# karfly/learnable-triangulation-pytorch

Hardware: AMD Instinct MI355X
Metric: multi-view samples/sec (4-view vol-softmax forward) (higher is better)
Workload: dtype bf16; 1 GPU; BASELINE config 2: volumetric-softmax forward, 4 views 384x384, 64^3 voxel cube, ResNet-152, random-init weights; per_gpu_batch=64, global_batch=64, parallelism=batch-sharded replicas x1, no data-path collective, hip_graph=True, self_launched=False

## Files before the change

include/lt_hip.h:

```cpp
#ifndef LT_HIP_H
#define LT_HIP_H

#include <stddef.h>
#include <stdint.h>

#ifdef __cplusplus
extern "C" {
#endif

#define LT_ABI_VERSION 1

enum { LT_F32 = 0, LT_BF16 = 1,
       LT_FP8 = 2  };
enum { LT_OK = 0, LT_ERR_INVALID = -1, LT_ERR_UNSUPPORTED = -2, LT_ERR_LAUNCH = -3 };

enum { LT_AGG_SUM = 0, LT_AGG_MAX = 1, LT_AGG_SOFTMAX = 2, LT_AGG_CONF = 3,
       LT_AGG_CONF_NORM = 4  };

enum {
    LT_EPI_RELU_PRE = 1,
    LT_EPI_RELU_POST = 2,
    LT_EPI_STORE_F32 = 4,
    LT_EPI_SIGMOID = 8,
    LT_EPI_RES_F32 = 64,
    LT_BN_FROZEN = 32,
    LT_BN_Y_BF16 = 128,
    LT_ACT_BF16 = 256
};

const char* lt_last_error(void);
int lt_abi_version(void);
int lt_device_info(int* cu_count, int* lds_per_cu, char* arch, int arch_len);

#define LT_CONV_MAX_PHASES 8

typedef struct lt_conv_phase {
    const void* weight;
    const int32_t* taps;
    int32_t ntaps;
    int32_t out_off[3];
    const void* weight_frag;
    int32_t weight_frag_layout;
} lt_conv_phase;

typedef struct lt_conv_desc {
    int32_t dtype;
    int32_t N, D, H, W, Cin;
    int32_t Do, Ho, Wo;
    int32_t stride[3], pad[3];
    int32_t OD, OH, OW;
    int32_t out_stride[3];
    int32_t Cout, ldc;
    int32_t cout_pad, k_pad;
    int32_t nphase;
    int32_t flags;
    int32_t tile;
    int32_t stages;
    lt_conv_phase phase[LT_CONV_MAX_PHASES];
} lt_conv_desc;

int lt_conv_pack_weights(const void* weight, int32_t cout_pad, int32_t k_pad, void* packed, void* stream);
int lt_conv_pack_weights_t32(const void* weight, int32_t cout_pad, int32_t k_pad, int32_t cin, int32_t ntaps, void* packed,
                             void* stream);
int lt_conv_pack_weights32(const void* weight, int32_t cout_pad, int32_t k_pad, void* packed, void* stream);

enum { LT_TILE_AUTO = 0,
       LT_TILE_128x128 = 1, LT_TILE_128x64 = 2, LT_TILE_256x32 = 3, LT_TILE_256x16 = 4, LT_TILE_64x64 = 5,
       LT_TILE2_128x128 = 11, LT_TILE2_128x64 = 12, LT_TILE2_256x32 = 13, LT_TILE2_256x16 = 14, LT_TILE2_64x64 = 15,
       LT_TILE_HALO = 20,
       LT_TILE3_288 = 30,
       LT_TILE_DIRECT = 99  };

int lt_conv_fwd(const lt_conv_desc* desc, const void* x, const float* bias, const float* scale, const float* shift,
                const void* residual, void* y, void* stream);
typedef struct lt_conv_skip {
    const void* x;
    int32_t cin;
    const void* weight_frag;
} lt_conv_skip;
int lt_conv_skip_fwd(const lt_conv_desc* desc, const void* x, const float* bias, const float* scale, const float* shift,
                     const lt_conv_skip* skip, void* y, void* stream);
typedef struct lt_conv_cat2 {
    const void* x;
    int32_t cin, H, W, stride;
} lt_conv_cat2;
int lt_conv_cat2_fwd(const lt_conv_desc* desc, const void* x, const lt_conv_cat2* second, const float* bias, const float* scale, const float* shift,
                     const void* residual, void* y, void* stream);
int lt_conv_cout_pad(int32_t cout);
int32_t lt_conv_chunk_samples(int32_t N, int64_t per_sample);

typedef struct lt_wshape {
    int32_t nd;
    int64_t s[5];
} lt_wshape;
int lt_sel_conv_skip(int32_t dtype, const int32_t x[5], const lt_wshape* w, const int32_t skip_x[5], const lt_wshape* skip_w);
int lt_sel_halo7_col(int32_t dtype, const int32_t x[5]);
int lt_sel_conv_cat2(int32_t dtype, const int32_t t2[5], const lt_wshape* w_expand, const int32_t x[5], const lt_wshape* w_down, int32_t stride_down);
int lt_sel_splitk_slices(const lt_conv_desc* d, const lt_wshape* w, int32_t transposed);
int lt_sel_bottleneck(int32_t dtype, const int32_t x[5], const lt_wshape w[3], const int32_t strides[3]);
int lt_sel_bottleneck_ds(int32_t dtype, const int32_t x[5], const lt_wshape w[3], const int32_t strides[3], const lt_wshape* w_down, int32_t stride_down);
int lt_sel_expand_reduce(int32_t dtype, const int32_t t2[5], const int32_t res[5], const lt_wshape* w_expand, const lt_wshape* w_reduce);
int lt_sel_stem_pool(int32_t dtype, const int32_t x[5], const lt_wshape* w, int32_t stride, int32_t pad, const int32_t pool[3]);
int lt_sel_pwchain(int32_t dtype, const int32_t x[5], int32_t nlayers, const lt_wshape* w);
int lt_sel_frag_layout(const lt_conv_desc* d, const lt_wshape* w, int32_t transposed, int32_t has_residual);

int lt_maxpool_fwd(int32_t dtype, const void* x, void* y, int32_t N, int32_t D, int32_t H, int32_t W, int32_t C,
                   const int32_t k[3], const int32_t s[3], const int32_t p[3], void* stream);

int lt_global_avgpool(int32_t dtype, const void* x, void* y, int32_t N, int32_t HW, int32_t C, void* stream);

int lt_nchw_to_nhwc(int32_t dtype, const float* x, void* y, int32_t N, int32_t C, int32_t HW, int32_t c_pad, void* stream);
int lt_nhwc_to_nchw_f32(int32_t dtype, const void* x, float* y, int32_t N, int32_t C, int32_t HW, int32_t ld, void* stream);

int lt_splitk_reduce(int32_t dtype, const float* partial, int32_t S, int64_t N, int64_t rows_per_sample, int32_t C, const float* bias,
                     const float* scale, const float* shift, const void* residual, void* y, int32_t flags, void* stream);

int lt_coord_volumes(const float* pos, const float* center, const float* rot, float step, int32_t B, int32_t V,
                     int32_t cmu_transfer, float* coords, void* stream);
int lt_rotate_points(const float* x, const float* rot, float* y, int64_t n, void* stream);

int lt_unproject_fwd(int32_t dtype, const void* feats, const float* proj, const float* coords, const float* conf,
                     void* out, int32_t B, int32_t NV, int32_t C, int32_t h, int32_t w, int32_t v0, int32_t v1,
                     int32_t v2, int32_t agg, void* stream);
int lt_unproject_grid_fwd(int32_t dtype, const void* feats, const float* proj, const float* pos, const float* center, const float* rot,
                          float step, int32_t cmu_transfer, float* coords_out, const float* conf, void* out, int32_t B, int32_t NV,
                          int32_t C, int32_t h, int32_t w, int32_t V, int32_t agg, void* stream);
int lt_unproject_masked_fwd(int32_t dtype, const void* feats, const float* proj, const float* coords, const float* conf, const uint8_t* view_mask,
                            void* out, int32_t B, int32_t NV, int32_t C, int32_t h, int32_t w, int32_t v0, int32_t v1, int32_t v2, int32_t agg,
                            void* stream);
int lt_unproject_grid_masked_fwd(int32_t dtype, const void* feats, const float* proj, const float* pos, const float* center, const float* rot,
                                 float step, int32_t cmu_transfer, float* coords_out, const float* conf, const uint8_t* view_mask, void* out,
                                 int32_t B, int32_t NV, int32_t C, int32_t h, int32_t w, int32_t V, int32_t agg, void* stream);
enum { LT_KIND_MPII = 0, LT_KIND_COCO = 1 };
int lt_cuboid_from_keypoints(const float* keypoints_3d, int32_t B, int32_t J, int32_t kind, double cuboid_side, float* pos, float* center,
                             void* stream);

size_t lt_softargmax3d_workspace(int32_t B, int32_t J, int64_t nvox);
int lt_softargmax3d_fwd(const float* logits, const float* coords, float mult, int32_t softmax, int32_t channels_last,
                        int32_t ld, float* kp, float* probs, int32_t B, int32_t J, int64_t nvox, void* workspace,
                        void* stream);
size_t lt_softargmax3d_stats_workspace(int32_t B, int32_t J, int64_t nvox);
int lt_softargmax3d_stats_fwd(const float* logits, const float* coords, float mult, int32_t softmax, int32_t channels_last, int32_t ld,
                              float* kp, float* probs, float* stats, int32_t* peak_index, int32_t B, int32_t J, int64_t nvox, void* workspace,
                              void* stream);

int lt_softargmax2d_fwd(const float* heatmaps, float mult, int32_t softmax, float* coords, float* probs, int32_t NJ,
                        int32_t h, int32_t w, void* stream);
int lt_softargmax2d_stats_fwd(const float* heatmaps, float mult, int32_t softmax, float* coords, float* probs, float* stats, int32_t* peak_index,
                              int32_t NJ, int32_t h, int32_t w, void* stream);
int lt_softargmax2d_bwd(const float* probs, const float* coords, const float* grad_coords, float mult, int32_t softmax, float* grad_heatmaps,
                        int32_t NJ, int32_t h, int32_t w, void* stream);
int lt_triangulate_dlt_bwd(const float* proj, const float* points, const float* conf, const float* grad_out, float* grad_points, float* grad_conf,
                           int32_t B, int32_t NV, int32_t J, void* stream);

size_t lt_unproject_bwd_workspace(int32_t B, int32_t NV, int32_t C, int32_t v0, int32_t v1, int32_t v2);
int lt_unproject_bwd(int32_t dtype, const void* feats, const float* proj, const float* coords, const float* conf, const float* grad_out,
                     float* grad_feats, float* grad_conf, int32_t B, int32_t NV, int32_t C, int32_t h, int32_t w, int32_t v0, int32_t v1,
                     int32_t v2, int32_t agg, void* workspace, size_t workspace_bytes, void* stream);
int lt_unproject_masked_bwd(int32_t dtype, const void* feats, const float* proj, const float* coords, const float* conf, const uint8_t* view_mask,
                            const float* grad_out, float* grad_feats, float* grad_conf, int32_t B, int32_t NV, int32_t C, int32_t h, int32_t w,
                            int32_t v0, int32_t v1, int32_t v2, int32_t agg, void* workspace, size_t workspace_bytes, void* stream);
int lt_softargmax3d_bwd(const float* probs, const float* coords, const float* kp, const float* grad_kp, const int32_t* gp_idx,
                        const float* gp_val, float multiplier, int32_t softmax, int32_t channels_last, float* grad_logits, int32_t B,
                        int32_t J, int64_t nvox, void* stream);
int lt_softargmax3d_bwd_dense(const float* probs, const float* coords, const float* kp, const float* grad_kp, const int32_t* gp_idx,
                              const float* gp_val, const float* gp_dense, float* workspace_bj, float multiplier, int32_t softmax,
                              int32_t channels_last, float* grad_logits, int32_t B, int32_t J, int64_t nvox, void* stream);
int lt_volumetric_ce_fwd(const float* coords, const float* probs, const float* keypoints_gt, const float* validity, float* terms,
                         int32_t* idx, float* grad_val, int32_t B, int32_t J, int64_t nvox, void* stream);
size_t lt_bn_stats_workspace(int64_t rows, int32_t C);
int lt_bn_stats_fwd(int32_t dtype, const void* x, int64_t rows, int32_t C, float* mean, float* var, float* running_mean,
                    float* running_var, float momentum, void* workspace, void* stream);

int lt_bn_act_fwd(const void* y , const float* mean, const float* var, const float* gamma, const float* beta, const void* residual, void* z,
                  void* z_bf16 , int64_t rows, int32_t C, float eps,
                  int32_t flags, void* stream);
size_t lt_bn_act_bwd_workspace(int64_t rows, int32_t C);
int lt_bn_act_bwd(const void* dz, const void* y , const void* residual, const float* mean, const float* var, const float* gamma, const float* beta,
                  void* dy, void* dy_bf16 , float* dgamma, float* dbeta, void* dres, int32_t accumulate_res,
                  int64_t rows, int32_t C, float eps, int32_t flags, void* workspace, void* stream);
int lt_act_bwd(const void* dz, const void* z, const void* residual, void* dy, void* dres, int32_t accumulate_res, int64_t total, int32_t flags,
               void* stream);
size_t lt_channel_sum_workspace(int64_t rows, int32_t C);
// ... 40 lines not shown
                       void* stream);
int lt_adam_step(float* param, const float* grad, float* exp_avg, float* exp_avg_sq, int64_t n, float lr, double beta1, double beta2, float eps,
                 float weight_decay, int32_t step, void* stream);

int lt_triangulate_dlt(const float* proj, const float* points, const float* conf, float* out, int32_t B, int32_t NV,
                       int32_t J, void* stream);
int lt_alg_tail_fwd(const float* keypoints_hm, const float* conf_raw, int32_t ld_conf, const float* proj, float scale_x, float scale_y,
                    float* keypoints_2d, float* confidences, float* keypoints_3d, int32_t B, int32_t NV, int32_t J, void* stream);
int lt_alg_tail_masked_fwd(const float* keypoints_hm, const float* conf_raw, int32_t ld_conf, const float* proj, float scale_x, float scale_y,
                           const uint8_t* view_mask, float* keypoints_2d, float* confidences, float* keypoints_3d, int32_t B, int32_t NV,
                           int32_t J, void* stream);
int lt_alg_tail_stats_fwd(const float* keypoints_hm, const float* conf_raw, int32_t ld_conf, const float* proj, float scale_x, float scale_y,
                          const uint8_t* view_mask, const float* stats2d, float* keypoints_2d, float* confidences, float* keypoints_3d,
                          float* cov2d_img, float* reproj_err, float* cov3d, int32_t B, int32_t NV, int32_t J, void* stream);
int lt_triangulate_dlt_stats(const float* proj, const float* points, const float* conf, const float* cov2d, const uint8_t* view_mask, float* out,
                             float* reproj_err, float* cov3d, int32_t B, int32_t NV, int32_t J, void* stream);

int lt_heatmap_argmax_nchw_f32(const float* heatmaps, int32_t ld, float* heatmaps_nchw, int64_t* indices, int64_t* keypoints,
                               int32_t N, int32_t J, int32_t h, int32_t w, int32_t image_h, int32_t image_w, void* stream);
int lt_triangulate_ransac(const float* proj, const int64_t* points, const int32_t* pairs, int32_t n_iters, double eps, int32_t direct_opt,
                          float* out_kp3d, uint8_t* out_inliers, int32_t B, int32_t NV, int32_t J, void* stream);

int lt_crop_resize_u8(const uint8_t* src, int64_t src_bytes, const int64_t* desc, const int64_t* desc_host, int32_t N, int32_t H, int32_t W,
                      const float* lut, float* out, void* stream);

int lt_undistort_crop_resize_u8(const uint8_t* src, int64_t src_bytes, const int64_t* desc, const int64_t* desc_host, const int16_t* maps,
                                int64_t maps_bytes, int32_t N, int32_t H, int32_t W, const float* lut, float* out, void* stream);

#define LT_PWCHAIN_MAX 3
typedef struct {
    int32_t dtype;
    int32_t nlayers;
    int64_t rows;
    int32_t cin;
    int32_t ldy;
    int32_t cout[LT_PWCHAIN_MAX];
    int32_t k_pad[LT_PWCHAIN_MAX];
    int32_t flags[LT_PWCHAIN_MAX];
    const void* weight[LT_PWCHAIN_MAX];
    const float* bias[LT_PWCHAIN_MAX];
    const float* scale[LT_PWCHAIN_MAX];
    const float* shift[LT_PWCHAIN_MAX];
    int64_t plane;
} lt_pwchain_desc;
int lt_pwchain_fwd(const lt_pwchain_desc* desc, const void* x, void* y, void* stream);

typedef struct {
    int32_t dtype;
    int32_t N, H, W;
    int32_t Cin, Cout;
    const void* weight;
    const float* bias;
    const float* scale;
    const float* shift;
    int32_t x_layout;
} lt_stem_desc;
size_t lt_stem_packed_bytes(void);
int lt_stem_pack_weights(const void* weight, int32_t k_pad, void* packed, void* stream);
int lt_stem_pool_fwd(const lt_stem_desc* desc, const void* x, void* y, void* stream);

typedef struct {
    int32_t dtype;
    int32_t N, H, W;
    int32_t C, P;
    const void* weight[3];
    const float* bias[3];
    const float* scale[3];
    const float* shift[3];
} lt_bneck_desc;
int lt_bottleneck_fwd(const lt_bneck_desc* desc, const void* x, void* y, void* stream);

typedef struct {
    int32_t dtype;
    int32_t N, H, W;
    int32_t Cin, P, C;
    const void* weight[4];
    const float* scale[4];
    const float* shift[4];
} lt_bneck_ds_desc;
int lt_bottleneck_ds_fwd(const lt_bneck_ds_desc* desc, const void* x, void* y, void* stream);

typedef struct {
    int32_t dtype;
    int32_t C, P;
    int64_t M;
    const void* weight[2];
    const float* scale[2];
    const float* shift[2];
    const float* consts;
} lt_xr_desc;
int lt_expand_reduce_fwd(const lt_xr_desc* desc, const void* t2, const void* residual, void* y, void* t1_next, void* stream);

int lt_graph_begin(void* stream);
int lt_graph_end(void* stream, void** graph_exec_out);
int lt_graph_launch(void* graph_exec, void* stream);
int lt_graph_destroy(void* graph_exec);
int lt_event_create(void** ev_out);
int lt_event_record(void* ev, void* stream);
int lt_event_elapsed_ms(void* ev_start, void* ev_stop, float* ms_out);
int lt_event_destroy(void* ev);

typedef struct lt_plan lt_plan;
typedef struct lt_named_tensor {
    const char* name;
    const float* data;
    int32_t ndim;
    int64_t shape[5];
} lt_named_tensor;
typedef struct lt_vol_plan_config {
    int32_t dtype;
    int32_t num_layers;
    int32_t style_caffe;
    int32_t num_joints;
    int32_t B, NV, H, W;
    int32_t volume_size;
    double cuboid_side;
    double volume_multiplier;
    int32_t volume_softmax;
    int32_t aggregation;
    int32_t transfer_cmu_to_human36m;
    int32_t use_graph;
} lt_vol_plan_config;
typedef struct lt_plan_info_t {
    int32_t launches;
    int32_t heatmap_h, heatmap_w;
    double flops;
    int64_t bytes_allocated;
    int32_t n_expand_reduce, n_bottleneck, n_bottleneck_ds, n_conv_cat2, n_conv2d_halo, n_pwchain, n_stem_pool, n_splitk, n_conv_skip;
    int32_t graph_captured;
    const float* logits;
    int32_t logits_planar;
} lt_plan_info_t;
int lt_plan_create_vol(const lt_vol_plan_config* cfg, const lt_named_tensor* weights, int32_t nweights, lt_plan** plan_out);
int lt_plan_forward_vol(lt_plan* plan, const float* images, const double* K_host, const double* R_host, const double* t_host, const double* base_points_host,
                        const double* rot_host, float* keypoints_3d, float* volumes, float* features, float* coord_volumes, float* vol_confidences, void* stream);
enum { LT_MODEL_ALG = 1, LT_MODEL_RANSAC = 2 };
typedef struct lt_alg_plan_config {
    int32_t model;
    int32_t dtype;
    int32_t num_layers;
    int32_t style_caffe;
    int32_t num_joints;
    int32_t B, NV, H, W;
    int32_t use_confidences;
    int32_t heatmap_softmax;
    double heatmap_multiplier;
    int32_t direct_optimization;
    double reprojection_error_epsilon;
    int32_t use_graph;
} lt_alg_plan_config;
int lt_plan_create_alg(const lt_alg_plan_config* cfg, const lt_named_tensor* weights, int32_t nweights, lt_plan** plan_out);
int lt_plan_forward_alg(lt_plan* plan, const float* images, const float* proj, float* keypoints_3d, void* keypoints_2d, float* heatmaps,
                        float* confidences, void* stream);
typedef struct lt_cascade_plan_config {
    lt_alg_plan_config alg;
    lt_vol_plan_config vol;
    int32_t kind;
} lt_cascade_plan_config;
int lt_plan_create_cascade(const lt_cascade_plan_config* cfg, const lt_named_tensor* alg_weights, int32_t n_alg, const lt_named_tensor* vol_weights,
                           int32_t n_vol, lt_plan** plan_out);
int lt_plan_forward_cascade(lt_plan* plan, const float* images, const double* K_host, const double* R_host, const double* t_host, const double* rot_host,
                            float* keypoints_3d, float* alg_keypoints_3d, float* base_points, float* volumes, float* features, float* coord_volumes,
                            float* vol_confidences, void* stream);
int lt_plan_set_view_mask(lt_plan* plan, const uint8_t* mask_host);
int lt_plan_set_keypoint_stats(lt_plan* plan, float* stats_dev, int32_t* peak_index_dev);
int lt_plan_set_alg_keypoint_stats(lt_plan* plan, float* stats2d_dev, int32_t* peak_index_dev, float* cov2d_img_dev, float* reproj_err_dev,
                                   float* cov3d_dev);
int lt_plan_info(const lt_plan* plan, lt_plan_info_t* info);
void lt_plan_destroy(lt_plan* plan);

#ifdef __cplusplus
}
#endif
#endif
```

learnable-triangulation-pytorch_amd/csrc/bneck.hip:

```cpp
#include <stdlib.h>

#include <type_traits>

#include "wave_prims.h"

using namespace lt;

namespace {

__device__ uint4 g_zero_page_b[2];

#ifdef LT_BNECK_TRACE
#define LT_BNECK_TRACE_WG 4096
__device__ unsigned long long g_bneck_trace[LT_BNECK_TRACE_WG * 4 * 8];
#define BN_STAMP(k)                                                                                                  \
    do {                                                                                                             \
        if (blockIdx.x < LT_BNECK_TRACE_WG && lane == 0) g_bneck_trace[(blockIdx.x * 4 + wave) * 8 + (k)] = clock64(); \
    } while (0)
#else
#define BN_STAMP(k)
#endif

struct BneckArgs {
    const bf16_t* x;
// ... 623 lines not shown
                }
                const int slot = (4 * cb + 2 * q + hk) ^ fsw(n31);
                *(uint4*)((lptr_t)(size_t)(lds0 + T2_OFF + px * RB + slot * 16)) = make_uint4(o[0], o[1], o[2], o[3]);
            }
        }
    }
    __syncthreads();

    {
        const unsigned a2 = lds0 + T2_OFF + n31 * RB + ((hk ^ fsw(n31)) << 4);
        unsigned xd[NPB][2];
#pragma unroll
        for (int pb = 0; pb < NPB; ++pb) {
            const int hpc = (2 * pb + prr + 1) * HPI + pcc + 1;
#pragma unroll
            for (int s2 = 0; s2 < 2; ++s2) xd[pb][s2] = lds0 + XS_OFF + hpc * 64 + (((2 * s2 + hk) ^ swz64(hpc)) << 4);
        }
        f32x16 acc[NPB], accd[NPB];
        static_for<0, NU3>([&](auto uc) {
            constexpr int u = decltype(uc)::value;
            constexpr int q = u / NUQ, k = u % NUQ;
            const int ob = wave + 4 * q;
            if constexpr (k == 0) {
#pragma unroll
                for (int pb = 0; pb < NPB; ++pb)
#pragma unroll
                    for (int e = 0; e < 16; ++e) { acc[pb][e] = 0.f; accd[pb][e] = 0.f; }
            }
            if constexpr (u + WD3 < NU3) wf3[(u + WD3) % (WD3 + 1)] = load_w3(u + WD3);
            V16 xb[NPB];
            if constexpr (k < GD) {
#pragma unroll
                for (int pb = 0; pb < NPB; ++pb) xb[pb].u = *(const uint4*)((lptr_t)(size_t)(xd[pb][k & 1] + (k >> 1) * STAGE));
#pragma unroll
                for (int pb = 0; pb < NPB; ++pb)
                    accd[pb] = __builtin_amdgcn_mfma_f32_32x32x16_bf16(wf3[u % (WD3 + 1)].h, xb[pb].h, accd[pb], 0, 0, 0);
            } else {
                constexpr int g = k - GD;
#pragma unroll
                for (int pb = 0; pb < NPB; ++pb) xb[pb].u = *(const uint4*)((lptr_t)(size_t)((a2 ^ (g << 5)) + pb * 32 * RB));
#pragma unroll
                for (int pb = 0; pb < NPB; ++pb)
                    acc[pb] = __builtin_amdgcn_mfma_f32_32x32x16_bf16(wf3[u % (WD3 + 1)].h, xb[pb].h, acc[pb], 0, 0, 0);
            }
            __builtin_amdgcn_sched_barrier(0);
            if constexpr (k == NUQ - 1) {
#pragma unroll
                for (int j = 0; j < 2; ++j) {
                    float esc[8], esf[8], dsc[8], dsf[8];
#pragma unroll
                    for (int e = 0; e < 8; ++e) {
                        esc[e] = csel(cst3, 128 * q, 8 * j + e);
                        esf[e] = csel(cst3, 128 * q + 32, 8 * j + e);
                        dsc[e] = csel(cst3, 128 * q + 64, 8 * j + e);
                        dsf[e] = csel(cst3, 128 * q + 96, 8 * j + e);
                    }
#pragma unroll
                    for (int pb = 0; pb < NPB; ++pb) {
                        unsigned o[4];
#pragma unroll
                        for (int d = 0; d < 4; ++d) {
                            const int e = 2 * d;
                            const float r0 = accd[pb][8 * j + e] * dsc[e] + dsf[e], r1 = accd[pb][8 * j + e + 1] * dsc[e + 1] + dsf[e + 1];
                            const float v0 = fmaxf(acc[pb][8 * j + e] * esc[e] + esf[e] + r0, 0.f);
                            const float v1 = fmaxf(acc[pb][8 * j + e + 1] * esc[e + 1] + esf[e + 1] + r1, 0.f);
                            o[d] = pack_bf16x2(v0, v1);
                        }
                        *(uint4*)(a.y + poff[pb] + 32 * ob + 16 * j) = make_uint4(o[0], o[1], o[2], o[3]);
                    }
                }
            }
        });
    }
}

int launch_bneck_ds(const BneckDsArgs& a, hipStream_t s) {
    constexpr int lds = 180 * 128 + 2 * 180 * 64 + 128 * 128;
    static_assert(lds <= 80 * 1024, "two workgroups per CU");
    auto kern = bneck_ds_kernel<64, 64, 256>;
    LT_OPT_IN_LDS(kern, lds);
    const long long nblk = (long long)a.N * a.tiles_x * a.tiles_y;
    hipLaunchKernelGGL(kern, dim3((unsigned)nblk), dim3(256), lds, s, a);
    LT_CHECK_LAUNCH("lt_bottleneck_ds_fwd");
    return LT_OK;
}

}

#ifdef LT_BNECK_TRACE
extern "C" int lt_bneck_trace_read(void* host, int nbytes) {
    return (int)hipMemcpyFromSymbol(host, HIP_SYMBOL(g_bneck_trace), nbytes, 0, hipMemcpyDeviceToHost);
}
#endif

extern "C" int lt_bottleneck_fwd(const lt_bneck_desc* d, const void* x, void* y, void* stream) {
    LT_REQUIRE(d && x && y, LT_ERR_INVALID, "lt_bottleneck_fwd: null argument");
    LT_REQUIRE(x != y, LT_ERR_INVALID, "lt_bottleneck_fwd: in-place is not possible (neighbouring tiles read each other's halo)");
    LT_REQUIRE(d->dtype == LT_BF16, LT_ERR_UNSUPPORTED, "lt_bottleneck_fwd: bf16 only");
    LT_REQUIRE((d->C == 256 && d->P == 64) || (d->C == 512 && d->P == 128), LT_ERR_UNSUPPORTED,
               "lt_bottleneck_fwd: widths %d / %d (256 / 64 and 512 / 128: the identity blocks of ResNet layer1 / layer2)", d->C, d->P);
    LT_REQUIRE(d->N > 0 && d->H > 0 && d->W > 0 && d->H % 8 == 0 && d->W % 16 == 0, LT_ERR_UNSUPPORTED,
               "lt_bottleneck_fwd: map %d x %d (8 x 16 pixel tiles)", d->H, d->W);
    LT_REQUIRE((long long)d->N * d->H * d->W * d->C < (1ll << 31), LT_ERR_UNSUPPORTED, "lt_bottleneck_fwd: 32-bit element offsets");
    BneckArgs a;
    a.x = (const bf16_t*)x;
    a.y = (bf16_t*)y;
    a.w1 = (const bf16_t*)d->weight[0];
    a.w2 = (const bf16_t*)d->weight[1];
    a.w3 = (const bf16_t*)d->weight[2];
    for (int i = 0; i < 3; ++i) {
        LT_REQUIRE(d->weight[i] && d->scale[i] && d->shift[i], LT_ERR_INVALID, "lt_bottleneck_fwd: layer %d: null weight / scale / shift", i);
        a.bias[i] = d->bias[i];
        a.scale[i] = d->scale[i];
        a.shift[i] = d->shift[i];
    }
    a.N = d->N; a.H = d->H; a.W = d->W;
    a.tiles_x = d->W / 16; a.tiles_y = d->H / 8;
    hipStream_t s = (hipStream_t)stream;
#ifndef LT_BNECK_HELD64
#define LT_BNECK_HELD64 2
#endif
#ifndef LT_BNECK_HELD128
#define LT_BNECK_HELD128 1
#endif
    if (d->P == 64) return launch_bneck<256, 64, 4, LT_BNECK_HELD64>(a, s);
    return launch_bneck<512, 128, 3, LT_BNECK_HELD128>(a, s);
}

extern "C" int lt_bottleneck_ds_fwd(const lt_bneck_ds_desc* d, const void* x, void* y, void* stream) {
    LT_REQUIRE(d && x && y, LT_ERR_INVALID, "lt_bottleneck_ds_fwd: null argument");
    LT_REQUIRE(x != y, LT_ERR_INVALID, "lt_bottleneck_ds_fwd: in-place is not possible");
    LT_REQUIRE(d->dtype == LT_BF16, LT_ERR_UNSUPPORTED, "lt_bottleneck_ds_fwd: bf16 only");
    LT_REQUIRE(d->Cin == 64 && d->P == 64 && d->C == 256, LT_ERR_UNSUPPORTED,
               "lt_bottleneck_ds_fwd: widths %d -> %d -> %d (64 -> 64 -> 256: the first block of ResNet layer1)", d->Cin, d->P, d->C);
    LT_REQUIRE(d->N > 0 && d->H > 0 && d->W > 0 && d->H % 8 == 0 && d->W % 16 == 0, LT_ERR_UNSUPPORTED,
               "lt_bottleneck_ds_fwd: map %d x %d (8 x 16 pixel tiles)", d->H, d->W);
    LT_REQUIRE((long long)d->N * d->H * d->W * d->C < (1ll << 31), LT_ERR_UNSUPPORTED, "lt_bottleneck_ds_fwd: 32-bit element offsets");
    BneckDsArgs a;
    a.x = (const bf16_t*)x;
    a.y = (bf16_t*)y;
    for (int i = 0; i < 4; ++i) {
        LT_REQUIRE(d->weight[i] && d->scale[i] && d->shift[i], LT_ERR_INVALID, "lt_bottleneck_ds_fwd: layer %d: null weight / scale / shift", i);
        a.scale[i] = d->scale[i];
        a.shift[i] = d->shift[i];
    }
    a.w1 = (const bf16_t*)d->weight[0];
    a.w2 = (const bf16_t*)d->weight[1];
    a.w3 = (const bf16_t*)d->weight[2];
    a.wd = (const bf16_t*)d->weight[3];
    a.N = d->N; a.H = d->H; a.W = d->W;
    a.tiles_x = d->W / 16; a.tiles_y = d->H / 8;
    return launch_bneck_ds(a, (hipStream_t)stream);
}
```

learnable-triangulation-pytorch_amd/csrc/plan.hip:

```cpp
#include <math.h>
#include <stdlib.h>
#include <string.h>

#include <array>
#include <deque>
#include <functional>
#include <map>
#include <string>
#include <unordered_map>
#include <vector>

#include "lt_common.h"

using namespace lt;

namespace {

#define PL_TRY(call)                   \
    do {                               \
        const int rc_ = (call);        \
        if (rc_ != LT_OK) return rc_;  \
    } while (0)
#define PL_HIP(call)                                                        \
    do {                                                                    \
// ... 142 lines not shown
        const int o = (dims[i] - 1) * 2 - 2 * pd[i] + ks[i] + output_padding;
        LT_REQUIRE(o == 2 * dims[i], LT_ERR_UNSUPPORTED, "plan: a transposed convolution must exactly double the size (k = 4, p = 1 / k = 2, p = 0)");
        outs[i] = o;
    }
    const int cp = cout_pad_of(cout);
    struct DimPhase { int phi; std::vector<std::pair<int, int>> taps; };
    auto dim_phases = [&](int i) {
        std::vector<DimPhase> res;
        if (!nd3 && i == 0) { res.push_back({0, {{0, 0}}}); return res; }
        for (int phi = 0; phi < 2; ++phi) {
            DimPhase dp; dp.phi = phi;
            for (int kk = 0; kk < ks[i]; ++kk)
                if (floormod(phi + pd[i] - kk, 2) == 0) dp.taps.push_back({kk, floordiv(phi + pd[i] - kk, 2)});
            res.push_back(dp);
        }
        return res;
    };
    const int64_t ktot = (int64_t)kd * kh * kw;
    struct Raw { std::vector<std::pair<std::vector<float>, int>> dummy; };
    std::vector<PhaseSpec> phases;
    std::vector<std::vector<int>> phase_k;
    int ntaps_max = 0;
    for (const DimPhase& A : dim_phases(0))
        for (const DimPhase& Bp : dim_phases(1))
            for (const DimPhase& Cp : dim_phases(2)) {
                PhaseSpec ph; std::vector<int> kidx;
                for (auto& ta : A.taps)
                    for (auto& tb : Bp.taps)
                        for (auto& tc : Cp.taps) {
                            const int da = ta.second, db = tb.second, dc = tc.second;
                            ph.taps.push_back(da); ph.taps.push_back(db); ph.taps.push_back(dc); ph.taps.push_back(((da * Hh + db) * W + dc) * cin);
                            kidx.push_back((ta.first * kh + tb.first) * kw + tc.first);
                        }
                if (kidx.empty()) { ph.taps = {0, 0, 0, 0}; kidx.push_back(-1); }
                ph.ntaps = (int)kidx.size();
                ph.off[0] = A.phi; ph.off[1] = Bp.phi; ph.off[2] = Cp.phi;
                if (ph.ntaps > ntaps_max) ntaps_max = ph.ntaps;
                phases.push_back(ph); phase_k.push_back(kidx);
            }
    const int K = ntaps_max * cin, k_pad = (K + kstep - 1) / kstep * kstep;
    for (size_t p = 0; p < phases.size(); ++p) {
        PhaseSpec& ph = phases[p];
        ph.w.assign((size_t)cp * k_pad, 0.f);
        for (int t = 0; t < ph.ntaps; ++t) {
            const int kt = phase_k[p][t];
            if (kt < 0) continue;
            for (int ci = 0; ci < cin; ++ci)
                for (int co = 0; co < cout; ++co) ph.w[(size_t)co * k_pad + (size_t)t * cin + ci] = w.d[((int64_t)ci * cout + co) * ktot + kt];
        }
    }
    LT_REQUIRE((int)phases.size() <= LT_CONV_MAX_PHASES, LT_ERR_UNSUPPORTED, "plan: %d phases", (int)phases.size());
    sp.Cin = cin; sp.Do = D; sp.Ho = Hh; sp.Wo = W; sp.OD = outs[0]; sp.OH = outs[1]; sp.OW = outs[2];
    for (int i = 0; i < 3; ++i) { sp.st[i] = 1; sp.pd[i] = 0; }
    sp.ostr[0] = nd3 ? 2 : 1; sp.ostr[1] = 2; sp.ostr[2] = 2;
    sp.Cout = cout; sp.cout_pad = cp; sp.k_pad = k_pad;
    fold_bn(cout, bias, bn, cp, sp.bias, sp.scale, sp.shift);
    sp.ph = std::move(phases);
    return LT_OK;
}

}

struct lt_plan {
    lt_vol_plan_config cfg;
    int model = 0;
    lt_alg_plan_config acfg = {};
    const char* who = "lt_plan_create_vol";
    int dtype = LT_F32, es = 4;
    std::unordered_map<std::string, const lt_named_tensor*> sd;
    std::vector<void*> allocs;
    std::map<std::pair<size_t, int>, std::vector<char*>> pool;
    size_t bytes_alloc = 0;
    double flops = 0;
    typedef std::function<int(hipStream_t)> Op;
    std::vector<Op> ops;
    int npre = 0, ntail = 0;
    std::deque<lt_conv_desc> conv_descs;
    std::deque<lt_conv_skip> skip_descs;
    std::deque<lt_conv_cat2> cat2_descs;
    std::deque<lt_pwchain_desc> pw_descs;
    std::deque<lt_stem_desc> stem_descs;
    std::deque<lt_bneck_desc> bneck_descs;
    std::deque<lt_bneck_ds_desc> bneck_ds_descs;
    std::deque<lt_xr_desc> xr_descs;
    hipGraphExec_t graph = nullptr;
    bool captured = false;
    hipStream_t own_stream = nullptr; hipEvent_t own_ev[2] = {nullptr, nullptr};
    const float* cur_images = nullptr;
    float* out_kp = nullptr; float* out_probs = nullptr; float* out_feats = nullptr;
    const float* cur_proj = nullptr; void* out_kp2d = nullptr; float* out_hm = nullptr; float* out_conf = nullptr;
    float* geo_dev = nullptr; StagingRing geo; size_t n_geo = 0, o_pos = 0, o_cen = 0, o_rot = 0;
    Act feats, vol, logits, volc;
    float* coords = nullptr; float* kp = nullptr; float* probs = nullptr; void* sa_ws = nullptr;
    float* ks_stats = nullptr; int32_t* ks_index = nullptr; void* ks_ws = nullptr;
    float* aks_stats2d = nullptr; int32_t* aks_index = nullptr; float* aks_cov2d = nullptr; float* aks_reproj = nullptr; float* aks_cov3d = nullptr;
    Act algc;
    float* hm_nchw = nullptr; float* kp_hm = nullptr; int64_t* kp_i64 = nullptr;
    int hm_h = 0, hm_w = 0;
    lt_plan* sub_alg = nullptr; lt_plan* sub_vol = nullptr; int kind = 0;
    float* cproj_dev = nullptr; StagingRing cproj; float* ckp_alg = nullptr;
    bool masked = false, ran = false, mask_dirty = false;
    std::vector<uint8_t> mask_cur;
    const uint8_t* mask_dev = nullptr; size_t o_mask = 0;
    uint8_t* amask_dev = nullptr; StagingRing amask;
    int n_xr = 0, n_bneck = 0, n_bneck_ds = 0, n_cat2 = 0, n_halo2d = 0, n_pwchain = 0, n_stem = 0, n_splitk = 0, n_conv_skip = 0;

    ~lt_plan() {
        if (graph) (void)hipGraphExecDestroy(graph);
        if (own_stream) (void)hipStreamDestroy(own_stream);
        for (int i = 0; i < 2; ++i) if (own_ev[i]) (void)hipEventDestroy(own_ev[i]);
        for (void* p : allocs) (void)hipFree(p);
        delete sub_alg;
        delete sub_vol;
    }

    int dev_alloc(size_t bytes, void** out) {
        void* p = nullptr;
        PL_HIP(hipMalloc(&p, bytes ? bytes : 16));
        allocs.push_back(p);
        bytes_alloc += bytes;
        *out = p;
        return LT_OK;
    }
    int alloc(int n, int d, int h, int w, int c, int esz, Act& a) {
        a = Act(); a.n = n; a.d = d; a.h = h; a.w = w; a.c = c; a.es = esz;
        auto it = pool.find({a.bytes(), esz});
        if (it != pool.end() && !it->second.empty()) { a.p = it->second.back(); it->second.pop_back(); return LT_OK; }
        void* p; PL_TRY(dev_alloc(a.bytes(), &p)); a.p = (char*)p;
        return LT_OK;
    }
    void release(const Act& a) { if (a.p && a.pooled) pool[{a.bytes(), a.es}].push_back(a.p); }
    int upload(const void* host, size_t bytes, void** out) {
        PL_TRY(dev_alloc(bytes, out));
        PL_HIP(hipMemcpy(*out, host, bytes, hipMemcpyHostToDevice));
        return LT_OK;
    }
    int upload_f32(const std::vector<float>& v, const float** out) { void* p; PL_TRY(upload(v.data(), v.size() * 4, &p)); *out = (const float*)p; return LT_OK; }
    int upload_w(const std::vector<float>& v, const void** out) {
        if (es == 4) { void* p; PL_TRY(upload(v.data(), v.size() * 4, &p)); *out = p; return LT_OK; }
        std::vector<unsigned short> h(v.size());
        for (size_t i = 0; i < v.size(); ++i) h[i] = bf16_rne(v[i]);
        void* p; PL_TRY(upload(h.data(), h.size() * 2, &p)); *out = p;
        return LT_OK;
    }
    int upload_i32(const std::vector<int32_t>& v, const int32_t** out) { void* p; PL_TRY(upload(v.data(), v.size() * 4, &p)); *out = (const int32_t*)p; return LT_OK; }

    int get(const std::string& name, WT& w, int nd_expect = 0) {
        auto it = sd.find(name);
        LT_REQUIRE(it != sd.end(), LT_ERR_INVALID, "%s: state dict has no '%s'", who, name.c_str());
        const lt_named_tensor* t = it->second;
        LT_REQUIRE(t->data && t->ndim >= 1 && t->ndim <= 5 && (!nd_expect || t->ndim == nd_expect), LT_ERR_INVALID, "%s: '%s' has %d dimensions", who, name.c_str(), t->ndim);
        w.d = t->data; w.nd = t->ndim;
        for (int i = 0; i < t->ndim; ++i) w.s[i] = t->shape[i];
        return LT_OK;
    }
    bool has(const std::string& name) const { return sd.find(name) != sd.end(); }
    int get_vec(const std::string& name, int n, const float** out) {
        WT w; PL_TRY(get(name, w));
        LT_REQUIRE(w.numel() == n, LT_ERR_INVALID, "%s: '%s' has %lld elements, expected %d", who, name.c_str(), (long long)w.numel(), n);
        *out = w.d;
        return LT_OK;
    }
    int get_bn(const std::string& prefix, int c, BN& bn) {
        PL_TRY(get_vec(prefix + ".weight", c, &bn.g)); PL_TRY(get_vec(prefix + ".bias", c, &bn.b));
        PL_TRY(get_vec(prefix + ".running_mean", c, &bn.m)); PL_TRY(get_vec(prefix + ".running_var", c, &bn.v));
        return LT_OK;
    }

    struct ConvOpt {
        const float* bias = nullptr; const BN* bn = nullptr;
        int stride = 1, pad = 0; bool transposed = false, relu = false, relu_pre = false, out_f32 = false, sigmoid = false;
        const Act* residual = nullptr;
        const Act* skip_x = nullptr; const WT* skip_w = nullptr; const float* skip_bias = nullptr; const BN* skip_bn = nullptr;
    };

    void fill_desc(lt_conv_desc& d, const ConvSpec& sp) {
        memset(&d, 0, sizeof(d));
        d.dtype = dtype;
        d.N = sp.N; d.D = sp.D; d.H = sp.H; d.W = sp.W; d.Cin = sp.Cin; d.Do = sp.Do; d.Ho = sp.Ho; d.Wo = sp.Wo;
        for (int i = 0; i < 3; ++i) { d.stride[i] = sp.st[i]; d.pad[i] = sp.pd[i]; d.out_stride[i] = sp.ostr[i]; }
        d.OD = sp.OD; d.OH = sp.OH; d.OW = sp.OW;
        d.Cout = sp.Cout; d.ldc = sp.Cout; d.cout_pad = sp.cout_pad; d.k_pad = sp.k_pad;
        d.nphase = (int)sp.ph.size(); d.flags = sp.flags; d.tile = 0; d.stages = 0;
        for (size_t i = 0; i < sp.ph.size(); ++i) {
            d.phase[i].ntaps = sp.ph[i].ntaps;
            for (int k = 0; k < 3; ++k) d.phase[i].out_off[k] = sp.ph[i].off[k];
        }
    }
// ... 168 lines not shown
            const void* wdev; PL_TRY(upload_w(sp.ph[0].w, &wdev));
            const float *bi, *sc, *sh;
            PL_TRY(upload_f32(sp.bias, &bi)); PL_TRY(upload_f32(sp.scale, &sc)); PL_TRY(upload_f32(sp.shift, &sh));
            d.cout[i] = sp.Cout; d.k_pad[i] = sp.k_pad; d.flags[i] = fl; d.weight[i] = wdev; d.bias[i] = bi; d.scale[i] = sc; d.shift[i] = sh;
            flops += 2.0 * d.rows * sp.Cout * L[i].w.s[1];
            shape[4] = sp.Cout; cout_last = sp.Cout;
        }
        d.ldy = cout_last;
        const long long vox = (long long)x.d * x.h * x.w;
        const bool planar = vox % 64 == 0;
        if (planar) d.plane = vox;
        PL_TRY(alloc(x.n, x.d, x.h, x.w, cout_last, 4, y));
        y.planar = planar; y.pooled = !planar;
        const lt_pwchain_desc* dp = &d; const void* xp = x.p; void* yp = y.p;
        ops.push_back([=](hipStream_t s) { return lt_pwchain_fwd(dp, xp, yp, s); });
        ++n_pwchain;
        return LT_OK;
    }

    int maxpool(const Act& x, int k, int s, int p, int nd, Act& y) {
        int32_t kk[3] = {nd == 2 ? 1 : k, k, k}, ss[3] = {nd == 2 ? 1 : s, s, s}, pp[3] = {nd == 2 ? 0 : p, p, p};
        const int od = (x.d + 2 * pp[0] - kk[0]) / ss[0] + 1, oh = (x.h + 2 * pp[1] - kk[1]) / ss[1] + 1, ow = (x.w + 2 * pp[2] - kk[2]) / ss[2] + 1;
        PL_TRY(alloc(x.n, od, oh, ow, x.c, x.es, y));
        const int dt = dtype; const Act xa = x; void* yp = y.p;
        std::vector<int32_t> a = {kk[0], kk[1], kk[2], ss[0], ss[1], ss[2], pp[0], pp[1], pp[2]};
        ops.push_back([=](hipStream_t st) { return lt_maxpool_fwd(dt, xa.p, yp, xa.n, xa.d, xa.h, xa.w, xa.c, a.data(), a.data() + 3, a.data() + 6, st); });
        return LT_OK;
    }

    int global_avgpool(const Act& x, Act& y) {
        PL_TRY(alloc(1, 1, 1, x.n, x.c, x.es, y));
        const int dt = dtype; const Act xa = x; void* yp = y.p;
        ops.push_back([=](hipStream_t st) { return lt_global_avgpool(dt, xa.p, yp, xa.n, xa.d * xa.h * xa.w, xa.c, st); });
        return LT_OK;
    }

    int pack_block_layer(const WT& w, const BN& bn, const int in[5], int pad, int fl, const void** wfr, const float** sc, const float** sh, ConvSpec& sp) {
        PL_TRY(make_conv_spec(w, nullptr, &bn, in, 1, pad, es, false, fl, 0, sp));
        LT_REQUIRE(sp.cout_pad == sp.Cout && sp.k_pad == sp.ph[0].ntaps * sp.Cin, LT_ERR_INVALID, "plan: fused block layer padding (%d / %d)", sp.cout_pad, sp.k_pad);
        const void* wdev; PL_TRY(upload_w(sp.ph[0].w, &wdev));
        PL_TRY(pack_frag(wdev, (size_t)sp.cout_pad * sp.k_pad, 2, sp.cout_pad, sp.k_pad, sp.Cin, sp.ph[0].ntaps, wfr));
        PL_TRY(upload_f32(sp.scale, sc)); PL_TRY(upload_f32(sp.shift, sh));
        flops += 2.0 * in[0] * in[2] * in[3] * sp.Cout * sp.ph[0].ntaps * sp.Cin;
        return LT_OK;
    }
    int bottleneck(const Act& x, const WT w[3], const BN bn[3], Act& y) {
        PL_TRY(alloc(x.n, 1, x.h, x.w, x.c, es, y));
        bneck_descs.emplace_back();
        lt_bneck_desc& d = bneck_descs.back();
        memset(&d, 0, sizeof(d));
        d.dtype = dtype; d.N = x.n; d.H = x.h; d.W = x.w; d.C = x.c; d.P = (int)w[0].s[0];
        int shape[5] = {x.n, 1, x.h, x.w, x.c};
        for (int i = 0; i < 3; ++i) {
            ConvSpec sp;
            PL_TRY(pack_block_layer(w[i], bn[i], shape, i == 1 ? 1 : 0, LT_EPI_RELU_POST, &d.weight[i], &d.scale[i], &d.shift[i], sp));
            shape[4] = sp.Cout;
        }
        const lt_bneck_desc* dp = &d; const void* xp = x.p; void* yp = y.p;
        ops.push_back([=](hipStream_t s) { return lt_bottleneck_fwd(dp, xp, yp, s); });
        ++n_bneck;
        return LT_OK;
    }
    int bottleneck_ds(const Act& x, const WT w[3], const BN bn[3], const WT& wd, const BN& bnd, Act& y) {
        const int Cc = (int)w[2].s[0];
        PL_TRY(alloc(x.n, 1, x.h, x.w, Cc, es, y));
        bneck_ds_descs.emplace_back();
        lt_bneck_ds_desc& d = bneck_ds_descs.back();
        memset(&d, 0, sizeof(d));
        d.dtype = dtype; d.N = x.n; d.H = x.h; d.W = x.w; d.Cin = x.c; d.P = (int)w[0].s[0]; d.C = Cc;
        int shape[5] = {x.n, 1, x.h, x.w, x.c};
        for (int i = 0; i < 3; ++i) {
            ConvSpec sp;
            PL_TRY(pack_block_layer(w[i], bn[i], shape, i == 1 ? 1 : 0, LT_EPI_RELU_POST, &d.weight[i], &d.scale[i], &d.shift[i], sp));
            shape[4] = sp.Cout;
        }
        const int xs[5] = {x.n, 1, x.h, x.w, x.c};
        ConvSpec sp;
        PL_TRY(pack_block_layer(wd, bnd, xs, 0, 0, &d.weight[3], &d.scale[3], &d.shift[3], sp));
        const lt_bneck_ds_desc* dp = &d; const void* xp = x.p; void* yp = y.p;
        ops.push_back([=](hipStream_t s) { return lt_bottleneck_ds_fwd(dp, xp, yp, s); });
        ++n_bneck_ds;
        return LT_OK;
    }
    int expand_reduce(const Act& t2, const Act& res, const WT& we, const BN& bne, const WT& wr, const BN& bnr, Act& y, Act& t1) {
        const int N = t2.n, Hh = t2.h, W = t2.w, P = t2.c, Cc = res.c;
        PL_TRY(alloc(N, 1, Hh, W, Cc, es, y));
        PL_TRY(alloc(N, 1, Hh, W, P, es, t1));
        xr_descs.emplace_back();
        lt_xr_desc& d = xr_descs.back();
        memset(&d, 0, sizeof(d));
        d.dtype = dtype; d.C = Cc; d.P = P; d.M = (long long)N * Hh * W;
        const int s2[5] = {t2.n, 1, Hh, W, P}, sr[5] = {res.n, 1, Hh, W, Cc};
        ConvSpec s3, s1;
        PL_TRY(pack_block_layer(we, bne, s2, 0, LT_EPI_RELU_POST, &d.weight[0], &d.scale[0], &d.shift[0], s3));
        PL_TRY(pack_block_layer(wr, bnr, sr, 0, LT_EPI_RELU_POST, &d.weight[1], &d.scale[1], &d.shift[1], s1));
        std::vector<float> packed;
        packed.insert(packed.end(), s3.scale.begin(), s3.scale.end()); packed.insert(packed.end(), s3.shift.begin(), s3.shift.end());
        packed.insert(packed.end(), s1.scale.begin(), s1.scale.end()); packed.insert(packed.end(), s1.shift.begin(), s1.shift.end());
        PL_TRY(upload_f32(packed, &d.consts));
        const lt_xr_desc* dp = &d; const void* a = t2.p; const void* r = res.p; void* yp = y.p; void* tp = t1.p;
        ops.push_back([=](hipStream_t s) { return lt_expand_reduce_fwd(dp, a, r, yp, tp, s); });
        ++n_xr;
        return LT_OK;
    }
    int stem_pool(int N, int Hh, int W, const WT& w, const BN& bn, Act& y) {
        const int in[5] = {N, 1, Hh, W, 8};
        ConvSpec sp;
        PL_TRY(make_conv_spec(w, nullptr, &bn, in, 2, 3, es, false, LT_EPI_RELU_POST, 0, sp));
        const int Hp = (sp.Ho - 1) / 2 + 1, Wp = (sp.Wo - 1) / 2 + 1;
        PL_TRY(alloc(N, 1, Hp, Wp, 64, es, y));
        const void* wdev; PL_TRY(upload_w(sp.ph[0].w, &wdev));
        void* wpk; PL_TRY(dev_alloc(lt_stem_packed_bytes(), &wpk));
        PL_TRY(lt_stem_pack_weights(wdev, sp.k_pad, wpk, nullptr));
        PL_HIP(hipStreamSynchronize(nullptr));
        stem_descs.emplace_back();
        lt_stem_desc& d = stem_descs.back();
        memset(&d, 0, sizeof(d));
        d.dtype = dtype; d.N = N; d.H = Hh; d.W = W; d.Cin = 3; d.Cout = 64; d.weight = wpk; d.x_layout = 1;
        PL_TRY(upload_f32(sp.bias, &d.bias)); PL_TRY(upload_f32(sp.scale, &d.scale)); PL_TRY(upload_f32(sp.shift, &d.shift));
        flops += 2.0 * N * sp.Ho * sp.Wo * 64 * 49 * w.s[1];
        const lt_stem_desc* dp = &d; void* yp = y.p; lt_plan* self = this;
        LT_REQUIRE(ops.empty(), LT_ERR_INVALID, "plan: an op reading the caller's tensor must be the first of the plan");
        ops.push_back([=](hipStream_t s) { return lt_stem_pool_fwd(dp, self->cur_images, yp, s); });
        npre = 1;
        ++n_stem;
        return LT_OK;
    }

    struct Block {
        bool bottleneck; int nconv; WT w[3]; BN bn[3]; int strides[3]; bool has_ds; WT wd; BN bnd; int sds;
        bool identity_bottleneck() const { return bottleneck && !has_ds && strides[0] == 1 && strides[1] == 1 && strides[2] == 1; }
    };
    int load_block(const std::string& pre, bool bott, bool caffe, int stride, bool ds, Block& b) {
        b.bottleneck = bott; b.nconv = bott ? 3 : 2; b.has_ds = ds; b.sds = stride;
        if (bott) { b.strides[0] = caffe ? stride : 1; b.strides[1] = caffe ? 1 : stride; b.strides[2] = 1; }
        else { b.strides[0] = stride; b.strides[1] = 1; b.strides[2] = 1; }
        for (int i = 0; i < b.nconv; ++i) {
            PL_TRY(get(pre + ".conv" + std::to_string(i + 1) + ".weight", b.w[i], 4));
            PL_TRY(get_bn(pre + ".bn" + std::to_string(i + 1), (int)b.w[i].s[0], b.bn[i]));
        }
        if (ds) { PL_TRY(get(pre + ".downsample.0.weight", b.wd, 4)); PL_TRY(get_bn(pre + ".downsample.1", (int)b.wd.s[0], b.bnd)); }
        return LT_OK;
    }
    int record_block(const Block& b, const Act& x, const Act* t1_in, const Block* nxt, Act& y, Act& t1n) {
        t1n = Act();
        const lt_wshape w3[3] = {wshape(b.w[0]), wshape(b.w[1]), wshape(b.w[2])}, wd = wshape(b.wd);
        if (b.bottleneck && !b.has_ds && !t1_in && !nxt && lt_sel_bottleneck(dtype, dims(x).data(), w3, b.strides)) return bottleneck(x, b.w, b.bn, y);
        if (b.bottleneck && b.has_ds && !t1_in && !nxt && lt_sel_bottleneck_ds(dtype, dims(x).data(), w3, b.strides, &wd, b.sds))
            return bottleneck_ds(x, b.w, b.bn, b.wd, b.bnd, y);
        if (t1_in || nxt) {
            Act t1, t2;
            ConvOpt o;
            if (t1_in) t1 = *t1_in;
            else { o = ConvOpt(); o.bn = &b.bn[0]; o.relu = true; PL_TRY(conv(x, b.w[0], o, t1)); }
            o = ConvOpt(); o.bn = &b.bn[1]; o.relu = true; o.pad = 1; PL_TRY(conv(t1, b.w[1], o, t2));
            release(t1);
            const lt_wshape wr = nxt ? wshape(nxt->w[0]) : lt_wshape{};
            if (nxt && lt_sel_expand_reduce(dtype, dims(t2).data(), dims(x).data(), &w3[2], &wr)) {
                PL_TRY(expand_reduce(t2, x, b.w[2], b.bn[2], nxt->w[0], nxt->bn[0], y, t1n));
                release(t2);
                return LT_OK;
            }
            o = ConvOpt(); o.bn = &b.bn[2]; o.relu = true; o.residual = &x; PL_TRY(conv(t2, b.w[2], o, y));
            release(t2);
            return LT_OK;
        }
        if (b.bottleneck && b.has_ds) {
            const int Ho = (x.h - 1) / b.sds + 1, Wo = (x.w - 1) / b.sds + 1;
            const int t2s[5] = {x.n, 1, Ho, Wo, (int)b.w[2].s[1]};
            if (lt_sel_conv_cat2(dtype, t2s, &w3[2], dims(x).data(), &wd, b.sds)) {
                Act t1, t2; ConvOpt o;
                o.bn = &b.bn[0]; o.relu = true; o.stride = b.strides[0]; PL_TRY(conv(x, b.w[0], o, t1));
                o = ConvOpt(); o.bn = &b.bn[1]; o.relu = true; o.stride = b.strides[1]; o.pad = 1; PL_TRY(conv(t1, b.w[1], o, t2));
                release(t1);
                PL_TRY(conv_cat2(t2, b.w[2], b.bn[2], x, b.wd, b.bnd, b.sds, y));
                release(t2);
                return LT_OK;
            }
        }
        Act res = x; bool own_res = false;
        if (b.has_ds) { ConvOpt o; o.bn = &b.bnd; o.stride = b.sds; PL_TRY(conv(x, b.wd, o, res)); own_res = true; }
        Act cur = x;
        for (int i = 0; i < b.nconv; ++i) {
            const bool last = i + 1 == b.nconv;
            ConvOpt o; o.bn = &b.bn[i]; o.relu = true; o.stride = b.strides[i]; o.pad = (int)b.w[i].s[2] / 2; o.residual = last ? &res : nullptr;
            Act z; PL_TRY(conv(cur, b.w[i], o, z));
            if (cur.p != x.p) release(cur);
            cur = z;
        }
        if (own_res) release(res);
        y = cur;
        return LT_OK;
    }

    int record_gap_head(const std::string& pre, const Act& x, Act& out) {
        WT w0, w4; const float *b0, *b4; BN bn1, bn5;
        PL_TRY(get(pre + ".features.0.weight", w0, 4)); PL_TRY(get_vec(pre + ".features.0.bias", (int)w0.s[0], &b0)); PL_TRY(get_bn(pre + ".features.1", (int)w0.s[0], bn1));
        PL_TRY(get(pre + ".features.4.weight", w4, 4)); PL_TRY(get_vec(pre + ".features.4.bias", (int)w4.s[0], &b4)); PL_TRY(get_bn(pre + ".features.5", (int)w4.s[0], bn5));
        Act y, p, g;
        ConvOpt o; o.bias = b0; o.bn = &bn1; o.pad = 1; o.relu = true; PL_TRY(conv(x, w0, o, y));
        PL_TRY(maxpool(y, 2, 2, 0, 2, p)); release(y);
        o = ConvOpt(); o.bias = b4; o.bn = &bn5; o.pad = 1; o.relu = true; PL_TRY(conv(p, w4, o, y)); release(p);
        PL_TRY(maxpool(y, 2, 2, 0, 2, p)); release(y);
        PL_TRY(global_avgpool(p, g)); release(p);
        Act cur = g;
        for (int i = 0; i < 3; ++i) {
            WT lw; const float* lb;
            PL_TRY(get(pre + ".head." + std::to_string(2 * i) + ".weight", lw, 2));
            PL_TRY(get_vec(pre + ".head." + std::to_string(2 * i) + ".bias", (int)lw.s[0], &lb));
            lw.nd = 4; lw.s[2] = 1; lw.s[3] = 1;
            ConvOpt lo; lo.bias = lb; lo.relu = i < 2; lo.sigmoid = i == 2; lo.out_f32 = i == 2;
            Act z; PL_TRY(conv(cur, lw, lo, z)); release(cur);
            cur = z;
        }
        out = cur;
        return LT_OK;
    }

    int record_backbone(int N, int Hh, int W, int num_layers, bool caffe, const char* conf_head, bool want_heatmaps, Act& feats256, Act& conf, Act& heatmaps) {
        int nb[4]; bool bott;
        switch (num_layers) {
            case 18: bott = false; nb[0] = 2; nb[1] = 2; nb[2] = 2; nb[3] = 2; break;
            case 34: bott = false; nb[0] = 3; nb[1] = 4; nb[2] = 6; nb[3] = 3; break;
            case 50: bott = true; nb[0] = 3; nb[1] = 4; nb[2] = 6; nb[3] = 3; break;
            case 101: bott = true; nb[0] = 3; nb[1] = 4; nb[2] = 23; nb[3] = 3; break;
            case 152: bott = true; nb[0] = 3; nb[1] = 8; nb[2] = 36; nb[3] = 3; break;
            default: set_error("%s: num_layers %d (18 / 34 / 50 / 101 / 152)", who, num_layers); return LT_ERR_INVALID;
        }
        if (caffe) bott = true;
        const int exp = bott ? 4 : 1;
        WT w1; BN bn1;
        PL_TRY(get("backbone.conv1.weight", w1, 4)); PL_TRY(get_bn("backbone.bn1", 64, bn1));
        Act y;
        const int32_t stem_in[5] = {N, 1, Hh, W, 8}, pool[3] = {3, 2, 1};
        const lt_wshape ws1 = wshape(w1);
        if (w1.s[1] == 3 && lt_sel_stem_pool(dtype, stem_in, &ws1, 2, 3, pool)) PL_TRY(stem_pool(N, Hh, W, w1, bn1, y));
        else {
            const int cpad = 16 / es;
            Act xin; PL_TRY(alloc(N, 1, Hh, W, cpad, es, xin)); xin.pooled = false;
            const int dt = dtype; lt_plan* self = this; void* xp = xin.p;
            ops.push_back([=](hipStream_t s) { return lt_nchw_to_nhwc(dt, self->cur_images, xp, N, 3, Hh * W, cpad, s); });
            npre = 1;
            ConvOpt o; o.bn = &bn1; o.stride = 2; o.pad = 3; o.relu = true;
            Act c1; PL_TRY(conv(xin, w1, o, c1));
            PL_TRY(maxpool(c1, 3, 2, 1, 2, y)); release(c1);
        }
        int inplanes = 64;
        const int planes_of[4] = {64, 128, 256, 512};
        for (int li = 0; li < 4; ++li) {
// ... 543 lines not shown
    if (base_points) PL_HIP(hipMemcpyAsync(base_points, Vp->geo_dev + Vp->o_cen, (size_t)B * 3 * 4, hipMemcpyDeviceToDevice, st));
    Vp->cur_images = images; Vp->out_kp = keypoints_3d; Vp->out_probs = volumes; Vp->out_feats = features;
    PL_TRY(Vp->run(st));
    if (coord_volumes) PL_HIP(hipMemcpyAsync(coord_volumes, Vp->coords, (size_t)B * V * V * V * 3 * 4, hipMemcpyDeviceToDevice, st));
    if (vol_confidences) PL_HIP(hipMemcpyAsync(vol_confidences, Vp->volc.p, (size_t)B * NV * 32 * 4, hipMemcpyDeviceToDevice, st));
    PL_TRY(p->leave(st, detour));
    return LT_OK;
}

extern "C" int lt_plan_set_view_mask(lt_plan* p, const uint8_t* mask_host) {
    const char* who = "lt_plan_set_view_mask";
    LT_REQUIRE(p, LT_ERR_INVALID, "%s: null plan", who);
    LT_REQUIRE(p->model != LT_MODEL_RANSAC, LT_ERR_UNSUPPORTED, "%s: the plan is %s; RANSAC takes no view mask (its inlier search drops views per joint)", who,
               plan_kind_name(p));
    const int B = p->cfg.B, NV = p->cfg.NV;
    const int need = p->model == 0 ? 1 : 2;
    std::vector<uint8_t> m((size_t)B * NV, 1);
    for (size_t i = 0; mask_host && i < m.size(); ++i) m[i] = mask_host[i] ? 1 : 0;
    for (int b = 0; b < B; ++b) {
        int n = 0;
        for (int v = 0; v < NV; ++v) n += m[(size_t)b * NV + v];
        LT_REQUIRE(n >= need, LT_ERR_INVALID, "%s: sample %d has %d valid view%s, at least %d needed (%s)", who, b, n, n == 1 ? "" : "s", need, plan_kind_name(p));
    }
    if (!p->masked) {
        LT_REQUIRE(!p->ran, LT_ERR_INVALID, "%s: the first call must come before the plan's first forward (the recorded and captured launches are chosen "
                   "there); create a new plan for masked forwards", who);
        if (p->model == MODEL_CASCADE) {
            PL_TRY(p->sub_vol->grow_geometry_for_mask());
            p->sub_alg->mask_dev = p->sub_vol->mask_dev;
            p->sub_vol->masked = p->sub_alg->masked = true;
        } else if (p->model == 0) {
            PL_TRY(p->grow_geometry_for_mask());
        } else {
            PL_TRY(p->alloc_alg_mask());
        }
        p->masked = true;
    }
    lt_plan* holder = p->model == MODEL_CASCADE ? p->sub_vol : p;
    holder->mask_cur = m;
    holder->mask_dirty = true;
    return LT_OK;
}

extern "C" int lt_plan_set_keypoint_stats(lt_plan* p, float* stats_dev, int32_t* peak_index_dev) {
    const char* who = "lt_plan_set_keypoint_stats";
    LT_REQUIRE(p, LT_ERR_INVALID, "%s: null plan", who);
    LT_REQUIRE(p->model == 0 || p->model == MODEL_CASCADE, LT_ERR_UNSUPPORTED, "%s: the plan is %s; the statistics are those of the volumetric joints' 3D heatmaps", who,
               plan_kind_name(p));
    LT_REQUIRE((stats_dev == nullptr) == (peak_index_dev == nullptr), LT_ERR_INVALID, "%s: stats_dev and peak_index_dev come together (both NULL: the plain tail)", who);
    lt_plan* v = p->model == MODEL_CASCADE ? p->sub_vol : p;
    if (stats_dev && !v->ks_ws) {
        const int V = v->cfg.volume_size;
        PL_TRY(v->dev_alloc(lt_softargmax3d_stats_workspace(v->cfg.B, v->cfg.num_joints, (int64_t)V * V * V), &v->ks_ws));
    }
    v->ks_stats = stats_dev; v->ks_index = peak_index_dev;
    return LT_OK;
}

extern "C" int lt_plan_set_alg_keypoint_stats(lt_plan* p, float* stats2d_dev, int32_t* peak_index_dev, float* cov2d_img_dev, float* reproj_err_dev,
                                              float* cov3d_dev) {
    const char* who = "lt_plan_set_alg_keypoint_stats";
    LT_REQUIRE(p, LT_ERR_INVALID, "%s: null plan", who);
    LT_REQUIRE(p->model == LT_MODEL_ALG || p->model == MODEL_CASCADE, LT_ERR_UNSUPPORTED, "%s: the plan is %s; the statistics are those of the algebraic joints", who,
               plan_kind_name(p));
    const int n = (stats2d_dev != nullptr) + (peak_index_dev != nullptr) + (cov2d_img_dev != nullptr) + (reproj_err_dev != nullptr) + (cov3d_dev != nullptr);
    LT_REQUIRE(n == 0 || n == 5, LT_ERR_INVALID,
               "%s: stats2d_dev, peak_index_dev, cov2d_img_dev, reproj_err_dev and cov3d_dev come together (all NULL: the plain tail); %d of 5 given", who, n);
    lt_plan* a = p->model == MODEL_CASCADE ? p->sub_alg : p;
    a->aks_stats2d = stats2d_dev; a->aks_index = peak_index_dev; a->aks_cov2d = cov2d_img_dev; a->aks_reproj = reproj_err_dev; a->aks_cov3d = cov3d_dev;
    return LT_OK;
}

extern "C" int lt_plan_info(const lt_plan* p, lt_plan_info_t* info) {
    LT_REQUIRE(p && info, LT_ERR_INVALID, "lt_plan_info: null argument");
    memset(info, 0, sizeof(*info));
    if (p->model == MODEL_CASCADE) {
        lt_plan_info_t a;
        PL_TRY(lt_plan_info(p->sub_vol, info));
        PL_TRY(lt_plan_info(p->sub_alg, &a));
        info->launches += a.launches + 1;
        info->flops += a.flops; info->bytes_allocated += a.bytes_allocated + (int64_t)p->bytes_alloc;
        info->n_expand_reduce += a.n_expand_reduce; info->n_bottleneck += a.n_bottleneck; info->n_bottleneck_ds += a.n_bottleneck_ds; info->n_conv_cat2 += a.n_conv_cat2;
        info->n_conv2d_halo += a.n_conv2d_halo; info->n_pwchain += a.n_pwchain; info->n_stem_pool += a.n_stem_pool; info->n_splitk += a.n_splitk;
        info->n_conv_skip += a.n_conv_skip;
        info->graph_captured = (!p->sub_alg->cfg.use_graph || a.graph_captured) && (!p->sub_vol->cfg.use_graph || info->graph_captured) &&
                               (p->sub_alg->cfg.use_graph || p->sub_vol->cfg.use_graph) ? 1 : 0;
        return LT_OK;
    }
    info->launches = (int32_t)p->ops.size();
    info->heatmap_h = p->hm_h; info->heatmap_w = p->hm_w;
    info->flops = p->flops; info->bytes_allocated = (int64_t)p->bytes_alloc;
    info->n_expand_reduce = p->n_xr; info->n_bottleneck = p->n_bneck; info->n_bottleneck_ds = p->n_bneck_ds; info->n_conv_cat2 = p->n_cat2;
    info->n_conv2d_halo = p->n_halo2d; info->n_pwchain = p->n_pwchain; info->n_stem_pool = p->n_stem; info->n_splitk = p->n_splitk; info->n_conv_skip = p->n_conv_skip;
    info->graph_captured = p->captured ? 1 : 0;
    info->logits = (const float*)p->logits.p; info->logits_planar = p->logits.planar ? 1 : 0;
    return LT_OK;
}

extern "C" void lt_plan_destroy(lt_plan* p) { delete p; }
```

learnable-triangulation-pytorch_amd/csrc/select.hip:

```cpp
#include "conv_common.h"

using namespace lt;

namespace {

bool wshape_is(const lt_wshape* w, int nd, int64_t s0, int64_t s1, int64_t s2, int64_t s3, int64_t s4 = 0) {
    const int64_t s[5] = {s0, s1, s2, s3, s4};
    if (w->nd != nd) return false;
    for (int i = 0; i < nd; ++i)
        if (w->s[i] != s[i]) return false;
    return true;
}

bool pointwise(const lt_wshape* w) {
    for (int i = 2; i < w->nd; ++i)
        if (w->s[i] != 1) return false;
    return true;
}

}

extern "C" int lt_sel_conv_skip(int32_t dtype, const int32_t x[5], const lt_wshape* w, const int32_t skip_x[5], const lt_wshape* skip_w) {
    if (dtype != LT_BF16 || env_on("LT_NO_CONV_SKIP") || env_on("LT_HALO_NO_COL") || env_on("LT_HALO_NO_PERSIST") || env_on("LT_CONV_NO_HALO")) return 0;
    if (!wshape_is(w, 5, 32, 32, 3, 3, 3) || !wshape_is(skip_w, 5, 32, 16, 1, 1, 1)) return 0;
    const int N = x[0], D = x[1], H = x[2], W = x[3];
    if (x[4] != 32 || skip_x[0] != N || skip_x[1] != D || skip_x[2] != H || skip_x[3] != W || skip_x[4] != 16) return 0;
    const int nc = lt_conv_chunk_samples(N, (long long)D * H * W * 32);
    if (nc < 1) return 0;
    return halo_col_fits(nc, D, H, W) && halo_col_fits(N - (N - 1) / nc * nc, D, H, W);
}

extern "C" int lt_sel_halo7_col(int32_t dtype, const int32_t x[5]) {
    if (dtype != LT_BF16 || x[4] != 32 || env_on("LT_HALO_NO_COL7")) return 0;
    return halo7_col_fits(x[0], x[1], x[2], x[3]);
}

extern "C" int lt_sel_conv_cat2(int32_t dtype, const int32_t t2[5], const lt_wshape* we, const int32_t x[5], const lt_wshape* wd, int32_t s) {
    if (dtype != LT_BF16 || env_on("LT_NO_CONV_CAT2") || env_on("LT_CONV_NO_V7") || env_on("LT_CONV_NO_V3")) return 0;
    const int N = t2[0], Ho = t2[2], Wo = t2[3], P = t2[4];
    if (t2[1] != 1 || we->nd != 4 || wd->nd != 4 || !pointwise(we) || !pointwise(wd)) return 0;
    const long long Cc = we->s[0], Cin2 = wd->s[1];
    if (we->s[1] != P || wd->s[0] != Cc || (s != 1 && s != 2) || x[0] != N || x[1] != 1 || x[2] != Ho * s || x[3] != Wo * s || x[4] != Cin2) return 0;
    if (P % 32 || Cin2 % 32 || (P + Cin2) % 64 || Cc % 256 || (P & (P - 1))) return 0;
    const long long tiles = (((long long)N * Ho * Wo + 287) / 288) * (Cc / 256);
    if (tiles < 200 && !env_on("LT_CAT2_ANY_SIZE")) return 0;
    return (long long)N * Ho * Wo * Cc < (1ll << 31) && (long long)N * x[2] * x[3] * Cin2 < (1ll << 31);
}

extern "C" int lt_sel_splitk_slices(const lt_conv_desc* d, const lt_wshape* w, int32_t transposed) {
    if (d->dtype != LT_BF16 || transposed || (d->flags & (LT_EPI_STORE_F32 | LT_EPI_SIGMOID)) || env_on("LT_CONV_NO_SPLITK")) return 1;
    if (w->nd != 5 || w->s[2] != 3 || w->s[3] != 3 || w->s[4] != 3) return 1;
    for (int i = 0; i < 3; ++i)
        if (d->stride[i] != 1 || d->pad[i] != 1) return 1;
    if (d->Cin < 128 || d->Cin % 64 || d->Cout % 4 || d->Cout != d->cout_pad || d->D * d->H * d->W > 512) return 1;
    const long long rows = (long long)d->N * d->Do * d->Ho * d->Wo;
    const int bm = rows >= 8192 ? 128 : 64;
    const long long tiles = ((rows + bm - 1) / bm) * (d->cout_pad / bm);
    const long long S = 256 / tiles;
    return S > 8 ? 8 : S < 1 ? 1 : (int)S;
}

extern "C" int lt_sel_bottleneck(int32_t dtype, const int32_t x[5], const lt_wshape w[3], const int32_t strides[3]) {
    if (dtype != LT_BF16 || env_on("LT_NO_BNECK")) return 0;
    if (x[1] != 1 || strides[0] != 1 || strides[1] != 1 || strides[2] != 1) return 0;
    const int C = x[4];
    const int64_t P = w[0].s[0];
    if (!((C == 256 && P == 64) || (C == 512 && P == 128))) return 0;
    if (!wshape_is(&w[0], 4, P, C, 1, 1) || !wshape_is(&w[1], 4, P, P, 3, 3) || !wshape_is(&w[2], 4, C, P, 1, 1)) return 0;
    return x[2] % 8 == 0 && x[3] % 16 == 0 && (long long)x[0] * x[2] * x[3] * C < (1ll << 31);
}

extern "C" int lt_sel_bottleneck_ds(int32_t dtype, const int32_t x[5], const lt_wshape w[3], const int32_t strides[3], const lt_wshape* wd, int32_t sd) {
    if (dtype != LT_BF16 || env_on("LT_NO_BNECK") || env_on("LT_NO_BNECK_DS")) return 0;
    if (x[1] != 1 || strides[0] != 1 || strides[1] != 1 || strides[2] != 1 || sd != 1) return 0;
    if (x[4] != 64 || !wshape_is(&w[0], 4, 64, 64, 1, 1) || !wshape_is(&w[1], 4, 64, 64, 3, 3) || !wshape_is(&w[2], 4, 256, 64, 1, 1) ||
        !wshape_is(wd, 4, 256, 64, 1, 1))
        return 0;
    return x[2] % 8 == 0 && x[3] % 16 == 0 && (long long)x[0] * x[2] * x[3] * 256 < (1ll << 31);
}

extern "C" int lt_sel_expand_reduce(int32_t dtype, const int32_t t2[5], const int32_t res[5], const lt_wshape* we, const lt_wshape* wr) {
    if (dtype != LT_BF16 || env_on("LT_NO_XR")) return 0;
    if (t2[1] != 1 || res[1] != 1 || t2[0] != res[0] || t2[2] != res[2] || t2[3] != res[3] || res[4] != 1024 || t2[4] != 256) return 0;
    if ((long long)t2[0] * t2[2] * t2[3] < 36 * 96 && !env_on("LT_XR_ANY_SIZE")) return 0;
    return wshape_is(we, 4, 1024, 256, 1, 1) && wshape_is(wr, 4, 256, 1024, 1, 1);
}

extern "C" int lt_sel_stem_pool(int32_t dtype, const int32_t x[5], const lt_wshape* w, int32_t stride, int32_t pad, const int32_t pool[3]) {
    return dtype == LT_BF16 && x[1] == 1 && x[4] == 8 && w->nd == 4 && w->s[2] == 7 && w->s[3] == 7 && w->s[0] == 64 && w->s[1] <= 8 && stride == 2 &&
           pad == 3 && pool[0] == 3 && pool[1] == 2 && pool[2] == 1;
}

extern "C" int lt_sel_pwchain(int32_t dtype, const int32_t x[5], int32_t nlayers, const lt_wshape* w) {
    if (dtype != LT_BF16 || nlayers < 1 || nlayers > LT_PWCHAIN_MAX || x[4] != 32) return 0;
    if ((long long)x[0] * x[1] * x[2] * x[3] % 64) return 0;
    int64_t cin = 32;
    for (int i = 0; i < nlayers; ++i) {
        if (!pointwise(&w[i]) || w[i].s[1] != cin || w[i].s[0] > 32 || (i + 1 < nlayers && w[i].s[0] != 32)) return 0;
        cin = w[i].s[0];
    }
    return 1;
}

extern "C" int lt_sel_frag_layout(const lt_conv_desc* d, const lt_wshape* w, int32_t transposed, int32_t has_residual) {
    if (d->dtype != LT_BF16) return 0;
    const bool w3x3 = !transposed && wshape_is(w, 4, 256, 256, 3, 3) && d->W == 24;
    const bool w4x4t = transposed && wshape_is(w, 4, 256, 256, 4, 4) && !env_on("LT_DECONV_NO_H2D");
    if ((w3x3 || w4x4t) && d->tile == LT_TILE_AUTO && !has_residual && !env_on("LT_CONV_NO_H2D") && !env_on("LT_CONV_V1") &&
        ((long long)d->N * (d->H / 8) * (d->W / 24) >= 60 || env_on("LT_H2D_ANY_SIZE")) && halo2d_fits(conv_args_of(*d), d->cout_pad, d->nphase))
        return 2;
    if (d->cout_pad % 256 == 0 && d->k_pad % 64 == 0) {
        const bool short_pw = pointwise(w) && d->k_pad <= 256 && !transposed;
        return !env_on("LT_CONV_NO_V7") && !short_pw ? 3 : 1;
    }
    const bool wreg = wshape_is(w, 5, 64, 64, 3, 3, 3) || wshape_is(w, 5, 64, 32, 3, 3, 3) || wshape_is(w, 5, 128, 128, 3, 3, 3) || wshape_is(w, 5, 32, 16, 3, 3, 3);
    if (transposed || !wreg || d->Cin != w->s[1]) return 0;
    for (int i = 0; i < 3; ++i)
        if (d->stride[i] != 1 || d->pad[i] != 1) return 0;
    return 2;
}
```

learnable-triangulation-pytorch_amd/lt_engine.py:

```python
import ctypes as C
from collections import OrderedDict
from dataclasses import dataclass, field
from typing import List, Optional, Tuple

import numpy as np
import torch
import torch.nn as nn

import lt_hip as H

BN_EPS = 1e-5


def cout_pad_of(cout):
    if cout <= 16:
        return 16
    if cout <= 32:
        return 32
    if cout <= 64:
        return 64
    return (cout + 127) // 128 * 128


def conv_chunk_samples(N, per_sample):
# ... 98 lines not shown
        k_pad = (K + kstep - 1) // kstep * kstep
        wk = w.permute(0, 2, 3, 4, 1).reshape(cout, K)
        taps = [(a, b, c, ((a * Hh + b) * W + c) * cin_buf) for a in range(kd) for b in range(kh) for c in range(kw)]
        bi, sc, sh = fold_bn(cout, bias, bn, cp)
        spec = ConvSpec(N, D, Hh, W, cin_buf, Do, Ho, Wo, st, pd, Do, Ho, Wo, (1, 1, 1), cout, cp, k_pad, flags, bi, sc, sh)
        spec.phases.append(ConvPhaseSpec(_pad_k(wk, cp, k_pad), torch.tensor(taps, dtype=torch.int32).reshape(-1, 4), (0, 0, 0)))
        return spec
    cin, cout, kd, kh, kw = w.shape
    assert cin == cin_buf, "transposed conv input may not be channel padded"
    nd3 = weight.dim() == 5
    assert all(s == 2 for s in (st if nd3 else st[1:])), "only stride-2 transposed convolutions"
    ks = (kd, kh, kw)
    dims = (D, Hh, W)
    outs = []
    for i in range(3):
        if not nd3 and i == 0:
            outs.append(1)
        else:
            o = (dims[i] - 1) * 2 - 2 * pd[i] + ks[i] + output_padding
            assert o == 2 * dims[i], "transposed conv must exactly double the size (k=4,p=1 / k=2,p=0; with output_padding=1: k=3,p=1 / k=1,p=0 -- the input gradients of the stride-2 convolutions)"
            outs.append(o)
    cp = cout_pad_of(cout)

    def dim_phases(i):
        if not nd3 and i == 0:
            return [(0, [(0, 0)])]
        res = []
        for phi in (0, 1):
            res.append((phi, [(kk, (phi + pd[i] - kk) // 2) for kk in range(ks[i]) if (phi + pd[i] - kk) % 2 == 0]))
        return res

    phase_list = []
    ntaps_max = 0
    for pa, ta in dim_phases(0):
        for pb, tb in dim_phases(1):
            for pc, tc in dim_phases(2):
                taps, cols = [], []
                for (ka, da) in ta:
                    for (kb, db) in tb:
                        for (kc, dc) in tc:
                            taps.append((da, db, dc, ((da * Hh + db) * W + dc) * cin))
                            cols.append(w[:, :, ka, kb, kc].t())
                if not taps:
                    taps, cols = [(0, 0, 0, 0)], [torch.zeros(cout, cin)]
                wk = torch.cat(cols, dim=1)
                phase_list.append((wk, taps, (pa, pb, pc)))
                ntaps_max = max(ntaps_max, len(taps))
    K = ntaps_max * cin
    k_pad = (K + kstep - 1) // kstep * kstep
    bi, sc, sh = fold_bn(cout, bias, bn, cp)
    ostr = (2 if nd3 else 1, 2, 2)
    spec = ConvSpec(N, D, Hh, W, cin, D, Hh, W, (1, 1, 1), (0, 0, 0), outs[0], outs[1], outs[2], ostr, cout, cp, k_pad, flags, bi, sc, sh)
    for wk, taps, off in phase_list:
        spec.phases.append(ConvPhaseSpec(_pad_k(wk, cp, k_pad), torch.tensor(taps, dtype=torch.int32).reshape(-1, 4), off))
    assert len(spec.phases) <= H.MAX_PHASES
    return spec


def stage_images(x, act, stream):
    N, Cc, Hh, W = x.shape
    H.check(H.lib().lt_nchw_to_nhwc(H.dtype_code(act.t.dtype), x.data_ptr(), act.t.data_ptr(), N, Cc, Hh * W, act.t.shape[-1], stream), "lt_nchw_to_nhwc")


class Act:
    __slots__ = ("t", "pooled")

    def __init__(self, t):
        self.t = t
        self.pooled = True

    @property
    def shape(self):
        return tuple(self.t.shape)


class Recorder:

    dtype = torch.float32
    live_weights = False

    def _declines(self, *a, **k):
        return False

    can_conv_skip = can_conv_cat2 = can_chain_pointwise = can_bottleneck = can_bottleneck_ds = can_expand_reduce = can_stem_pool = _declines


class PlanBuilder(Recorder):

    def __init__(self, device, dtype, tile_override=0, dry_run=False, stages=0):
        self.device = torch.device(device)
        self.dry_run = dry_run
        if self.device.type != "cuda" and not dry_run:
            raise RuntimeError("liblt_hip plans run on the GPU only (device=%s); there is no CPU fallback" % device)
        self.lib = None if dry_run else H.lib()
        self.dtype = dtype
        self.code = H.dtype_code(dtype)
        self.out_dtype = torch.bfloat16 if dtype == torch.float8_e4m3fn else dtype
        self.ops = []
        self.keep = []
        self.pool = {}
        self.tile_override = tile_override
        self.stages = stages
        self.live_weights = False
        self.live_frag = False
        self.flops = 0
        self.bytes_alloc = 0
        self.ntail = 0
        self.npre = 0

    def alloc(self, shape, dtype=None):
        dtype = dtype or self.dtype
        n = int(np.prod(shape)) * esize(dtype)
        lst = self.pool.get((n, dtype))
        if lst:
            t = lst.pop().view(*shape)
        else:
            t = torch.empty(shape, dtype=dtype, device=self.device)
            self.bytes_alloc += n
        self.keep.append(t)
        return Act(t)

    def release(self, act):
        if act is None or not act.pooled:
            return
        t = act.t
        n = t.numel() * t.element_size()
        self.pool.setdefault((n, t.dtype), []).append(t.reshape(-1))

    def const(self, t, dtype=None):
        t = t.to(device=self.device, dtype=dtype or t.dtype).contiguous()
        self.keep.append(t)
        return t

    def _add(self, fn, kind="op", label="", flops=0, nbytes=0, info=None):
        meta = {"kind": kind, "label": label, "flops": flops, "bytes": nbytes}
        if self.dry_run:
            meta["info"] = info or {}
        self.last_info = info or {}
        self.ops.append((fn, meta))

    def _fusable(self):
        return not (self.live_weights or self.tile_override)

    def can_conv_skip(self, x_shape, weight, skip_shape, skip_weight):
        if not self._fusable():
            return False
        return bool(H.lib().lt_sel_conv_skip(self.code, H.dims(x_shape), H.wshape(weight), H.dims(skip_shape), H.wshape(skip_weight)))

    def _desc(self, spec):
        d = H.ConvDesc()
        d.dtype = self.code
        d.N, d.D, d.H, d.W, d.Cin = spec.N, spec.D, spec.H, spec.W, spec.Cin
        d.Do, d.Ho, d.Wo = spec.Do, spec.Ho, spec.Wo
        d.stride = H.i3(spec.stride); d.pad = H.i3(spec.pad)
        d.OD, d.OH, d.OW = spec.OD, spec.OH, spec.OW
        d.out_stride = H.i3(spec.out_stride)
        d.Cout, d.ldc, d.cout_pad, d.k_pad = spec.Cout, spec.Cout, spec.cout_pad, spec.k_pad
        d.nphase, d.flags, d.tile, d.stages = len(spec.phases), spec.flags, self.tile_override, self.stages
        for i, ph in enumerate(spec.phases):
            d.phase[i].ntaps = ph.taps.shape[0]; d.phase[i].out_off = H.i3(ph.out_off)
        return d

    def frag_layout(self, spec, weight, transposed, residual):
        if self.live_weights and not self.live_frag:
            return 0
        return H.lib().lt_sel_frag_layout(self._desc(spec), H.wshape(weight), int(transposed), int(residual))

# ... 193 lines not shown
        assert self.can_chain_pointwise(x, layers)
        N, D, Hh, W, _ = x.shape
        d = H.PwChainDesc()
        d.dtype, d.nlayers, d.rows, d.cin = self.code, len(layers), N * D * Hh * W, 32
        specs = []
        shape = x.shape
        flops = 0
        for i, (w, bias, bn, relu) in enumerate(layers):
            last = i + 1 == len(layers)
            flags = (H.EPI_RELU_POST if relu else 0) | (H.EPI_STORE_F32 if last else 0)
            spec = make_conv_spec(w, bias, bn, shape, 1, 0, self.dtype, False, flags)
            specs.append(spec)
            rows = lambda t: t if t.shape[0] >= 32 else torch.cat([t, t.new_zeros((32 - t.shape[0],) + tuple(t.shape[1:]))])
            wdev = self.const(rows(spec.phases[0].weight), self.dtype)
            bi, sc, sh = self.const(rows(spec.bias)), self.const(rows(spec.scale)), self.const(rows(spec.shift))
            d.cout[i], d.k_pad[i], d.flags[i] = spec.Cout, spec.k_pad, flags
            d.weight[i], d.bias[i], d.scale[i], d.shift[i] = wdev.data_ptr(), bi.data_ptr(), sc.data_ptr(), sh.data_ptr()
            flops += 2 * d.rows * spec.Cout * w.shape[1]
            shape = (N, D, Hh, W, spec.Cout)
        d.ldy = specs[-1].Cout
        planar = bool(planar) and (D * Hh * W) % 64 == 0
        if planar:
            d.plane = D * Hh * W
            y = Act(self.alloc((N, shape[-1], D, Hh, W), torch.float32).t.permute(0, 2, 3, 4, 1))
            y.pooled = False
        else:
            y = self.alloc(shape, torch.float32)
        self.keep.append(x.t)
        self.keep.append(d)
        self.flops += flops
        label = "pwchain " + "->".join(str(c) for c in [32] + [sp.Cout for sp in specs]) + " @" + "x".join(str(v) for v in (N, D, Hh, W))
        nbytes = x.t.numel() * x.t.element_size() + y.t.numel() * 4
        self._add(lambda s, d=d, xp=x.t.data_ptr(), yp=y.t.data_ptr(): H.check(self.lib.lt_pwchain_fwd(C.byref(d), xp, yp, s), "lt_pwchain_fwd"),
                  "pwchain", label, flops, nbytes, {"specs": specs, "x": x, "y": y})
        return y

    def can_bottleneck(self, x, convs, strides):
        if not self._fusable() or len(convs) != 3:
            return False
        return bool(H.lib().lt_sel_bottleneck(self.code, H.dims(x.shape), (H.WShape * 3)(*map(H.wshape, convs)), H.i3(strides)))

    def bottleneck(self, x, convs, bns):
        assert self.can_bottleneck(x, convs, (1, 1, 1))
        return self._bneck(x, convs, bns)

    def _bneck(self, x, convs, bns, down=None):
        N, _, Hh, W, Cin = x.shape
        P, Cc = convs[0].shape[0], convs[2].shape[0]
        y = self.alloc((N, 1, Hh, W, Cc))
        if down is None:
            d = H.BneckDesc()
            d.dtype, d.N, d.H, d.W, d.C, d.P = self.code, N, Hh, W, Cc, P
        else:
            d = H.BneckDsDesc()
            d.dtype, d.N, d.H, d.W, d.Cin, d.P, d.C = self.code, N, Hh, W, Cin, P, Cc
        flops0, specs, shape = self.flops, [], x.shape
        for i, (w, bn) in enumerate(zip(convs, bns)):
            spec, d.weight[i], d.scale[i], d.shift[i] = self._pack_layer(w, bn, shape, 1 if i == 1 else 0, H.EPI_RELU_POST)
            specs.append(spec)
            shape = (N, 1, Hh, W, spec.Cout)
        if down is not None:
            spec, d.weight[3], d.scale[3], d.shift[3] = self._pack_layer(*down, x.shape, 0, 0)
            specs.append(spec)
        self.keep += [x.t, d]
        flops = self.flops - flops0
        esz = x.t.element_size()
        nbytes = (x.t.numel() + y.t.numel()) * esz + sum(sp.phases[0].weight.numel() for sp in specs) * esz
        name, fwd = ("bneck", "lt_bottleneck_fwd") if down is None else ("bneck-ds", "lt_bottleneck_ds_fwd")
        label = "%s %d->%d->%d @%s" % (name, Cin, P, Cc, "x".join(str(v) for v in (N, 1, Hh, W)))
        self._add(lambda s, d=d, xp=x.t.data_ptr(), yp=y.t.data_ptr(): H.check(getattr(self.lib, fwd)(C.byref(d), xp, yp, s), fwd),
                  "conv", label, flops, nbytes, {name.replace("-", "_"): True, "specs": specs, "x": x, "y": y})
        return y

    def can_bottleneck_ds(self, x, convs, strides, w_down, stride_down):
        if not self._fusable() or len(convs) != 3:
            return False
        return bool(H.lib().lt_sel_bottleneck_ds(self.code, H.dims(x.shape), (H.WShape * 3)(*map(H.wshape, convs)), H.i3(strides), H.wshape(w_down),
                                                  stride_down))

    def bottleneck_ds(self, x, convs, bns, w_down, bn_down):
        assert self.can_bottleneck_ds(x, convs, (1, 1, 1), w_down, 1)
        return self._bneck(x, convs, bns, (w_down, bn_down))

    def can_expand_reduce(self, t2, res, w_expand, w_reduce):
        if not self._fusable():
            return False
        return bool(H.lib().lt_sel_expand_reduce(self.code, H.dims(t2.shape), H.dims(res.shape), H.wshape(w_expand), H.wshape(w_reduce)))

    def expand_reduce(self, t2, res, w_expand, bn_expand, w_reduce, bn_reduce):
        assert self.can_expand_reduce(t2, res, w_expand, w_reduce)
        N, _, Hh, W, P = t2.shape
        Cc = res.shape[-1]
        y = self.alloc((N, 1, Hh, W, Cc))
        t1 = self.alloc((N, 1, Hh, W, P))
        d = H.XrDesc()
        d.dtype, d.C, d.P, d.M = self.code, Cc, P, N * Hh * W
        flops0 = self.flops
        s3, d.weight[0], d.scale[0], d.shift[0] = self._pack_layer(w_expand, bn_expand, t2.shape, 0, H.EPI_RELU_POST)
        s1, d.weight[1], d.scale[1], d.shift[1] = self._pack_layer(w_reduce, bn_reduce, res.shape, 0, H.EPI_RELU_POST)
        packed = self.const(torch.cat([s3.scale, s3.shift, s1.scale, s1.shift]))
        d.consts = packed.data_ptr()
        self.keep += [t2.t, res.t, d]
        flops = self.flops - flops0
        esz = t2.t.element_size()
        nbytes = (t2.t.numel() + res.t.numel() + y.t.numel() + t1.t.numel() + 2 * Cc * P) * esz
        label = "xr expand %d->%d + reduce %d->%d @%s" % (P, Cc, Cc, P, "x".join(str(v) for v in (N, 1, Hh, W)))
        self._add(lambda s, d=d, a=t2.t.data_ptr(), r=res.t.data_ptr(), yp=y.t.data_ptr(), tp=t1.t.data_ptr():
                  H.check(self.lib.lt_expand_reduce_fwd(C.byref(d), a, r, yp, tp, s), "lt_expand_reduce_fwd"),
                  "conv", label, flops, nbytes, {"xr": True, "specs": [s3, s1], "x": t2, "res": res, "y": y, "t1": t1})
        return y, t1

    def can_stem_pool(self, x, weight, stride, pad, pool):
        return bool(H.lib().lt_sel_stem_pool(self.code, H.dims(x.shape), H.wshape(weight), stride, pad, H.i3(pool)))

    def stem_pool(self, x, weight, bn, image_cell=None):
        assert self.can_stem_pool(x, weight, 2, 3, (3, 2, 1))
        if self.dry_run or weight.shape[1] != 3:
            image_cell = None
        assert image_cell is None or not self.ops, "an op reading the caller's tensor must be the first of the plan"
        N, _, Hh, W, _ = x.shape
        spec = make_conv_spec(weight, None, bn, x.shape, 2, 3, self.dtype, False, H.EPI_RELU_POST)
        Hp, Wp = (spec.Ho - 1) // 2 + 1, (spec.Wo - 1) // 2 + 1
        y = self.alloc((N, 1, Hp, Wp, 64))
        wdev = self.const(spec.phases[0].weight, self.dtype)
        bi, sc, sh = self.const(spec.bias), self.const(spec.scale), self.const(spec.shift)
        wpk = torch.empty(57344 if self.dry_run else self.lib.lt_stem_packed_bytes(), dtype=torch.uint8, device=self.device)
        if not self.dry_run:
            H.check(self.lib.lt_stem_pack_weights(wdev.data_ptr(), spec.k_pad, wpk.data_ptr(), H.cur_stream()), "lt_stem_pack_weights")
            torch.cuda.current_stream().synchronize()
        d = H.StemDesc()
        d.dtype, d.N, d.H, d.W, d.Cin, d.Cout = self.code, N, Hh, W, (3 if image_cell is not None else 8), 64
        d.weight, d.bias, d.scale, d.shift = wpk.data_ptr(), bi.data_ptr(), sc.data_ptr(), sh.data_ptr()
        d.x_layout = 1 if image_cell is not None else 0
        self.keep.append(x.t)
        self.keep.append(d)
        self.keep.append(wpk)
        flops = 2 * N * spec.Ho * spec.Wo * 64 * 49 * weight.shape[1]
        self.flops += flops
        esz = x.t.element_size()
        if image_cell is not None:
            def launch(s, d=d, yp=y.t.data_ptr(), cell=image_cell):
                if not cell.get("ptr"):
                    raise RuntimeError("stem_pool: the plan reads the caller's images; set image_cell['ptr'] before Plan.run")
                H.check(self.lib.lt_stem_pool_fwd(C.byref(d), cell["ptr"], yp, s), "lt_stem_pool_fwd")
            nbytes = N * 3 * Hh * W * 4 + y.t.numel() * esz + spec.phases[0].weight.numel() * esz
            self.npre += 1
        else:
            def launch(s, d=d, xp=x.t.data_ptr(), yp=y.t.data_ptr()):
                H.check(self.lib.lt_stem_pool_fwd(C.byref(d), xp, yp, s), "lt_stem_pool_fwd")
            nbytes = (x.t.numel() + y.t.numel()) * esz + spec.phases[0].weight.numel() * esz
        self._add(launch, "stem", "stem conv7x7/2+pool3x3/2 %d->64 @%s" % (d.Cin, "x".join(str(v) for v in (N, Hh, W))), flops, nbytes,
                  {"spec": spec, "x": x, "y": y})
        return y

    def maxpool(self, x, k, s, p, nd):
        N, D, Hh, W, Cc = x.shape
        kk = (1, k, k) if nd == 2 else (k, k, k)
        ss = (1, s, s) if nd == 2 else (s, s, s)
        pp = (0, p, p) if nd == 2 else (p, p, p)
        od = [(dim + 2 * pp[i] - kk[i]) // ss[i] + 1 for i, dim in enumerate((D, Hh, W))]
        y = self.alloc((N, od[0], od[1], od[2], Cc))
        self.keep.append(x.t)
        self._add(lambda st, xp=x.t.data_ptr(), yp=y.t.data_ptr(), a=(N, D, Hh, W, Cc), kk=H.i3(kk), ss=H.i3(ss), pp=H.i3(pp):
                  H.check(self.lib.lt_maxpool_fwd(self.code, xp, yp, a[0], a[1], a[2], a[3], a[4], kk, ss, pp, st), "lt_maxpool_fwd"),
                  "maxpool", "maxpool%dd k%d @%s" % (nd, k, "x".join(map(str, x.shape))), 0,
                  (x.t.numel() + y.t.numel()) * x.t.element_size(), {"x": x, "y": y, "k": kk, "s": ss, "p": pp})
# ... 118 lines not shown
```

learnable-triangulation-pytorch_amd/lt_hip.py:

```python
import ctypes as C
import os

import torch

HERE = os.path.dirname(os.path.abspath(__file__))
LIB_PATH = os.environ.get("LT_HIP_LIB") or os.path.join(HERE, "lib", "liblt_hip.so")

LT_F32, LT_BF16, LT_FP8 = 0, 1, 2
AGG = {"sum": 0, "max": 1, "softmax": 2, "conf": 3, "conf_norm": 4}
LT_MODEL_ALG, LT_MODEL_RANSAC = 1, 2
LT_KIND_MPII, LT_KIND_COCO = 0, 1
KIND = {"mpii": LT_KIND_MPII, "coco": LT_KIND_COCO}
EPI_RELU_PRE, EPI_RELU_POST, EPI_STORE_F32, EPI_SIGMOID = 1, 2, 4, 8
EPI_RES_F32 = 64
BN_FROZEN = 32
BN_Y_BF16 = 128
ACT_BF16 = 256
TILE_AUTO, TILE_128x128, TILE_128x64, TILE_256x32, TILE_256x16, TILE_64x64, TILE_DIRECT = 0, 1, 2, 3, 4, 5, 99
TILE2_128x128, TILE2_128x64, TILE2_256x32, TILE2_256x16, TILE2_64x64 = 11, 12, 13, 14, 15
TILE_HALO = 20
TILE3_288 = 30
MAX_PHASES = 8

vp, i32, i64, f32, f64 = C.c_void_p, C.c_int32, C.c_int64, C.c_float, C.c_double


class ConvPhase(C.Structure):
    _fields_ = [("weight", vp), ("taps", vp), ("ntaps", i32), ("out_off", i32 * 3), ("weight_frag", vp), ("weight_frag_layout", i32)]


class ConvDesc(C.Structure):
    _fields_ = [("dtype", i32), ("N", i32), ("D", i32), ("H", i32), ("W", i32), ("Cin", i32),
                ("Do", i32), ("Ho", i32), ("Wo", i32), ("stride", i32 * 3), ("pad", i32 * 3),
                ("OD", i32), ("OH", i32), ("OW", i32), ("out_stride", i32 * 3),
                ("Cout", i32), ("ldc", i32), ("cout_pad", i32), ("k_pad", i32),
                ("nphase", i32), ("flags", i32), ("tile", i32), ("stages", i32),
                ("phase", ConvPhase * MAX_PHASES)]


class ConvSkip(C.Structure):
    _fields_ = [("x", vp), ("cin", i32), ("weight_frag", vp)]


class ConvCat2(C.Structure):
    _fields_ = [("x", vp), ("cin", i32), ("H", i32), ("W", i32), ("stride", i32)]


class WShape(C.Structure):
    _fields_ = [("nd", i32), ("s", i64 * 5)]


def wshape(t):
    return WShape(t.dim(), (i64 * 5)(*t.shape))


def dims(shape):
    return (i32 * 5)(*shape)


PWCHAIN_MAX = 3


class PwChainDesc(C.Structure):
    _fields_ = [("dtype", i32), ("nlayers", i32), ("rows", i64), ("cin", i32), ("ldy", i32),
                ("cout", i32 * PWCHAIN_MAX), ("k_pad", i32 * PWCHAIN_MAX), ("flags", i32 * PWCHAIN_MAX),
                ("weight", vp * PWCHAIN_MAX), ("bias", vp * PWCHAIN_MAX), ("scale", vp * PWCHAIN_MAX), ("shift", vp * PWCHAIN_MAX),
                ("plane", i64)]


class StemDesc(C.Structure):
    _fields_ = [("dtype", i32), ("N", i32), ("H", i32), ("W", i32), ("Cin", i32), ("Cout", i32),
                ("weight", vp), ("bias", vp), ("scale", vp), ("shift", vp), ("x_layout", i32)]


class BneckDesc(C.Structure):
    _fields_ = [("dtype", i32), ("N", i32), ("H", i32), ("W", i32), ("C", i32), ("P", i32),
                ("weight", vp * 3), ("bias", vp * 3), ("scale", vp * 3), ("shift", vp * 3)]


class BneckDsDesc(C.Structure):
    _fields_ = [("dtype", i32), ("N", i32), ("H", i32), ("W", i32), ("Cin", i32), ("P", i32), ("C", i32),
                ("weight", vp * 4), ("scale", vp * 4), ("shift", vp * 4)]


class XrDesc(C.Structure):
    _fields_ = [("dtype", i32), ("C", i32), ("P", i32), ("M", C.c_int64), ("weight", vp * 2), ("scale", vp * 2), ("shift", vp * 2), ("consts", vp)]


class NamedTensor(C.Structure):
    _fields_ = [("name", C.c_char_p), ("data", vp), ("ndim", i32), ("shape", C.c_int64 * 5)]


class VolPlanConfig(C.Structure):
    _fields_ = [("dtype", i32), ("num_layers", i32), ("style_caffe", i32), ("num_joints", i32), ("B", i32), ("NV", i32), ("H", i32), ("W", i32),
                ("volume_size", i32), ("cuboid_side", C.c_double), ("volume_multiplier", C.c_double), ("volume_softmax", i32), ("aggregation", i32),
                ("transfer_cmu_to_human36m", i32), ("use_graph", i32)]


class AlgPlanConfig(C.Structure):
    _fields_ = [("model", i32), ("dtype", i32), ("num_layers", i32), ("style_caffe", i32), ("num_joints", i32), ("B", i32), ("NV", i32), ("H", i32),
                ("W", i32), ("use_confidences", i32), ("heatmap_softmax", i32), ("heatmap_multiplier", C.c_double), ("direct_optimization", i32),
                ("reprojection_error_epsilon", C.c_double), ("use_graph", i32)]


class CascadePlanConfig(C.Structure):
    _fields_ = [("alg", AlgPlanConfig), ("vol", VolPlanConfig), ("kind", i32)]


class PlanInfo(C.Structure):
    _fields_ = [("launches", i32), ("heatmap_h", i32), ("heatmap_w", i32), ("flops", C.c_double), ("bytes_allocated", C.c_int64),
                ("n_expand_reduce", i32), ("n_bottleneck", i32), ("n_bottleneck_ds", i32), ("n_conv_cat2", i32), ("n_conv2d_halo", i32), ("n_pwchain", i32),
                ("n_stem_pool", i32), ("n_splitk", i32), ("n_conv_skip", i32), ("graph_captured", i32), ("logits", vp), ("logits_planar", i32)]


SIGNATURES = {
    "lt_plan_create_vol": (C.c_int, [C.POINTER(VolPlanConfig), C.POINTER(NamedTensor), i32, C.POINTER(vp)]),
    "lt_plan_forward_vol": (C.c_int, [vp, vp, vp, vp, vp, vp, vp, vp, vp, vp, vp, vp, vp]),
    "lt_plan_create_alg": (C.c_int, [C.POINTER(AlgPlanConfig), C.POINTER(NamedTensor), i32, C.POINTER(vp)]),
    "lt_plan_forward_alg": (C.c_int, [vp, vp, vp, vp, vp, vp, vp, vp]),
    "lt_plan_create_cascade": (C.c_int, [C.POINTER(CascadePlanConfig), C.POINTER(NamedTensor), i32, C.POINTER(NamedTensor), i32, C.POINTER(vp)]),
    "lt_plan_forward_cascade": (C.c_int, [vp, vp, vp, vp, vp, vp, vp, vp, vp, vp, vp, vp, vp, vp]),
    "lt_plan_set_view_mask": (C.c_int, [vp, vp]),
    "lt_plan_set_keypoint_stats": (C.c_int, [vp, vp, vp]),
    "lt_plan_set_alg_keypoint_stats": (C.c_int, [vp, vp, vp, vp, vp, vp]),
    "lt_plan_info": (C.c_int, [vp, C.POINTER(PlanInfo)]),
    "lt_plan_destroy": (None, [vp]),
    "lt_last_error": (C.c_char_p, []),
    "lt_abi_version": (C.c_int, []),
    "lt_device_info": (C.c_int, [C.POINTER(C.c_int), C.POINTER(C.c_int), C.c_char_p, C.c_int]),
    "lt_conv_fwd": (C.c_int, [C.POINTER(ConvDesc), vp, vp, vp, vp, vp, vp, vp]),
    "lt_conv_skip_fwd": (C.c_int, [C.POINTER(ConvDesc), vp, vp, vp, vp, C.POINTER(ConvSkip), vp, vp]),
    "lt_conv_cat2_fwd": (C.c_int, [C.POINTER(ConvDesc), vp, C.POINTER(ConvCat2), vp, vp, vp, vp, vp, vp]),
    "lt_conv_cout_pad": (C.c_int, [i32]),
    "lt_conv_chunk_samples": (i32, [i32, i64]),
    "lt_sel_conv_skip": (C.c_int, [i32, i32 * 5, C.POINTER(WShape), i32 * 5, C.POINTER(WShape)]),
    "lt_sel_halo7_col": (C.c_int, [i32, i32 * 5]),
    "lt_sel_conv_cat2": (C.c_int, [i32, i32 * 5, C.POINTER(WShape), i32 * 5, C.POINTER(WShape), i32]),
    "lt_sel_splitk_slices": (C.c_int, [C.POINTER(ConvDesc), C.POINTER(WShape), i32]),
    "lt_sel_bottleneck": (C.c_int, [i32, i32 * 5, WShape * 3, i32 * 3]),
    "lt_sel_bottleneck_ds": (C.c_int, [i32, i32 * 5, WShape * 3, i32 * 3, C.POINTER(WShape), i32]),
    "lt_sel_expand_reduce": (C.c_int, [i32, i32 * 5, i32 * 5, C.POINTER(WShape), C.POINTER(WShape)]),
    "lt_sel_stem_pool": (C.c_int, [i32, i32 * 5, C.POINTER(WShape), i32, i32, i32 * 3]),
    "lt_sel_pwchain": (C.c_int, [i32, i32 * 5, i32, C.POINTER(WShape)]),
    "lt_sel_frag_layout": (C.c_int, [C.POINTER(ConvDesc), C.POINTER(WShape), i32, i32]),
    "lt_conv_pack_weights": (C.c_int, [vp, i32, i32, vp, vp]),
    "lt_conv_pack_weights_t32": (C.c_int, [vp, i32, i32, i32, i32, vp, vp]),
    "lt_conv_pack_weights32": (C.c_int, [vp, i32, i32, vp, vp]),
    "lt_pwchain_fwd": (C.c_int, [C.POINTER(PwChainDesc), vp, vp, vp]),
    "lt_stem_pool_fwd": (C.c_int, [C.POINTER(StemDesc), vp, vp, vp]),
    "lt_bottleneck_fwd": (C.c_int, [C.POINTER(BneckDesc), vp, vp, vp]),
    "lt_bottleneck_ds_fwd": (C.c_int, [C.POINTER(BneckDsDesc), vp, vp, vp]),
    "lt_expand_reduce_fwd": (C.c_int, [C.POINTER(XrDesc), vp, vp, vp, vp, vp]),
    "lt_stem_packed_bytes": (C.c_size_t, []),
    "lt_stem_pack_weights": (C.c_int, [vp, i32, vp, vp]),
    "lt_maxpool_fwd": (C.c_int, [i32, vp, vp, i32, i32, i32, i32, i32, i32 * 3, i32 * 3, i32 * 3, vp]),
    "lt_global_avgpool": (C.c_int, [i32, vp, vp, i32, i32, i32, vp]),
    "lt_nchw_to_nhwc": (C.c_int, [i32, vp, vp, i32, i32, i32, i32, vp]),
    "lt_nhwc_to_nchw_f32": (C.c_int, [i32, vp, vp, i32, i32, i32, i32, vp]),
    "lt_coord_volumes": (C.c_int, [vp, vp, vp, f32, i32, i32, i32, vp, vp]),
    "lt_rotate_points": (C.c_int, [vp, vp, vp, i64, vp]),
    "lt_unproject_fwd": (C.c_int, [i32, vp, vp, vp, vp, vp, i32, i32, i32, i32, i32, i32, i32, i32, i32, vp]),
    "lt_unproject_grid_fwd": (C.c_int, [i32, vp, vp, vp, vp, vp, f32, i32, vp, vp, vp, i32, i32, i32, i32, i32, i32, i32, vp]),
    "lt_unproject_masked_fwd": (C.c_int, [i32, vp, vp, vp, vp, vp, vp, i32, i32, i32, i32, i32, i32, i32, i32, i32, vp]),
    "lt_unproject_grid_masked_fwd": (C.c_int, [i32, vp, vp, vp, vp, vp, f32, i32, vp, vp, vp, vp, i32, i32, i32, i32, i32, i32, i32, vp]),
    "lt_cuboid_from_keypoints": (C.c_int, [vp, i32, i32, i32, C.c_double, vp, vp, vp]),
    "lt_softargmax3d_workspace": (C.c_size_t, [i32, i32, i64]),
    "lt_softargmax3d_fwd": (C.c_int, [vp, vp, f32, i32, i32, i32, vp, vp, i32, i32, i64, vp, vp]),
    "lt_softargmax3d_stats_workspace": (C.c_size_t, [i32, i32, i64]),
    "lt_softargmax3d_stats_fwd": (C.c_int, [vp, vp, f32, i32, i32, i32, vp, vp, vp, vp, i32, i32, i64, vp, vp]),
    "lt_softargmax2d_fwd": (C.c_int, [vp, f32, i32, vp, vp, i32, i32, i32, vp]),
    "lt_softargmax2d_stats_fwd": (C.c_int, [vp, f32, i32, vp, vp, vp, vp, i32, i32, i32, vp]),
    "lt_triangulate_dlt": (C.c_int, [vp, vp, vp, vp, i32, i32, i32, vp]),
    "lt_alg_tail_fwd": (C.c_int, [vp, vp, i32, vp, f32, f32, vp, vp, vp, i32, i32, i32, vp]),
    "lt_alg_tail_masked_fwd": (C.c_int, [vp, vp, i32, vp, f32, f32, vp, vp, vp, vp, i32, i32, i32, vp]),
    "lt_alg_tail_stats_fwd": (C.c_int, [vp, vp, i32, vp, f32, f32, vp, vp, vp, vp, vp, vp, vp, vp, i32, i32, i32, vp]),
    "lt_triangulate_dlt_stats": (C.c_int, [vp, vp, vp, vp, vp, vp, vp, vp, i32, i32, i32, vp]),
    "lt_heatmap_argmax_nchw_f32": (C.c_int, [vp, i32, vp, vp, vp, i32, i32, i32, i32, i32, i32, vp]),
    "lt_triangulate_ransac": (C.c_int, [vp, vp, vp, i32, C.c_double, i32, vp, vp, i32, i32, i32, vp]),
    "lt_crop_resize_u8": (C.c_int, [vp, i64, vp, vp, i32, i32, i32, vp, vp, vp]),
    "lt_undistort_crop_resize_u8": (C.c_int, [vp, i64, vp, vp, vp, i64, i32, i32, i32, vp, vp, vp]),
    "lt_bn_act_fwd": (C.c_int, [vp, vp, vp, vp, vp, vp, vp, vp, i64, i32, f32, i32, vp]),
    "lt_bn_act_bwd_workspace": (C.c_size_t, [i64, i32]),
    "lt_bn_act_bwd": (C.c_int, [vp, vp, vp, vp, vp, vp, vp, vp, vp, vp, vp, vp, i32, i64, i32, f32, i32, vp, vp]),
    "lt_act_bwd": (C.c_int, [vp, vp, vp, vp, vp, i32, i64, i32, vp]),
    "lt_channel_sum_workspace": (C.c_size_t, [i64, i32]),
    "lt_channel_sum": (C.c_int, [vp, i64, i32, vp, i32, vp, vp]),
    "lt_channel_sum_dt": (C.c_int, [i32, vp, i64, i32, vp, i32, vp, vp]),
    "lt_maxpool_bwd_dt": (C.c_int, [i32, vp, vp, vp, i32, i32, i32, i32, i32, i32 * 3, i32 * 3, i32 * 3, vp]),
    "lt_convert_pad": (C.c_int, [i32, vp, i32, vp, i64, i32, i32, vp]),
    "lt_maxpool_bwd": (C.c_int, [vp, vp, vp, i32, i32, i32, i32, i32, i32 * 3, i32 * 3, i32 * 3, vp]),
    "lt_adam_step_multi": (C.c_int, [vp, i32, i32, f64, f64, f32, f32, i32, vp]),
    "lt_add_f32": (C.c_int, [vp, vp, i64, vp]),
    "lt_pad_channels_f32": (C.c_int, [vp, vp, i64, i32, i32, vp]),
    "lt_zero": (C.c_int, [vp, i64, vp]),
    "lt_softargmax2d_bwd": (C.c_int, [vp, vp, vp, C.c_float, i32, vp, i32, i32, i32, vp]),
    "lt_triangulate_dlt_bwd": (C.c_int, [vp, vp, vp, vp, vp, vp, i32, i32, i32, vp]),
    "lt_splitk_reduce": (C.c_int, [i32, vp, i32, i64, i64, i32, vp, vp, vp, vp, vp, i32, vp]),
    "lt_add_i64_multi": (C.c_int, [vp, i32, i64, vp]),
    "lt_cast_f32_bf16": (C.c_int, [vp, vp, i64, vp]),
    "lt_gather_f32_multi": (C.c_int, [vp, i32, i32, vp]),
    "lt_amax_f32": (C.c_int, [vp, i64, vp, vp]),
    "lt_amax_dt": (C.c_int, [i32, vp, i64, vp, vp]),
    "lt_quant_fp8_dt": (C.c_int, [i32, vp, vp, i64, vp, vp, vp]),
    "lt_quant_fp8": (C.c_int, [vp, vp, i64, vp, vp, vp]),
    "lt_gather_f32_fp8": (C.c_int, [vp, vp, vp, i64, vp, vp, vp]),
    "lt_scale_product": (C.c_int, [vp, i32, vp, vp, vp]),
    "lt_gather_f32": (C.c_int, [vp, vp, vp, i64, vp]),
    "lt_gather_f32_bf16": (C.c_int, [vp, vp, vp, i64, vp]),
    "lt_conv_wgrad_workspace": (C.c_size_t, [i64, i32, i32]),
    "lt_pack_n8_bf16_bytes": (C.c_size_t, [i32, i64, i32]),
    "lt_pack_n8_bf16": (C.c_int, [vp, vp, i32, i64, i32, i32, vp]),
    "lt_pack_n8_from_bf16": (C.c_int, [vp, vp, i32, i64, i32, i32, vp]),
    "lt_conv_wgrad_bf16_workspace": (C.c_size_t, [i64, i32, i32]),
    "lt_conv_wgrad_bf16": (C.c_int, [vp, vp, vp, vp, i32, i32, i32, i32, i32, i32, i32, i32, i32 * 3, i32 * 3, i32, i32, i32, i32, i32, i32, vp, vp]),
    "lt_conv_wgrad_bf16_nhwc_ok": (C.c_int, [i32, i32, i32, i32, i32, i32, i32, i32, i32, i32 * 3, i32 * 3, i32, i32, i32, i32, i32]),
    "lt_conv_wgrad_bf16_nhwc": (C.c_int, [vp, vp, vp, vp, i32, i32, i32, i32, i32, i32, i32, i32, i32, i32 * 3, i32 * 3, i32, i32, i32, i32, i32, i32, vp, vp]),
    "lt_conv_wgrad": (C.c_int, [vp, vp, vp, vp, i32, i32, i32, i32, i32, i32, i32, i32, i32 * 3, i32 * 3, i32, i32, i32, i32, i32, i32, vp, vp]),
    "lt_adam_step": (C.c_int, [vp, vp, vp, vp, i64, f32, f64, f64, f32, f32, i32, vp]),
    "lt_unproject_bwd_workspace": (C.c_size_t, [i32, i32, i32, i32, i32, i32]),
    "lt_unproject_bwd": (C.c_int, [i32, vp, vp, vp, vp, vp, vp, vp, i32, i32, i32, i32, i32, i32, i32, i32, i32, vp, C.c_size_t, vp]),
    "lt_unproject_masked_bwd": (C.c_int, [i32, vp, vp, vp, vp, vp, vp, vp, vp, i32, i32, i32, i32, i32, i32, i32, i32, i32, vp, C.c_size_t, vp]),
    "lt_global_avgpool_bwd": (C.c_int, [vp, vp, i32, i32, i32, i32, vp]),
    "lt_global_avgpool_bwd_dt": (C.c_int, [i32, vp, vp, i32, i32, i32, i32, vp]),
    "lt_softargmax3d_bwd": (C.c_int, [vp, vp, vp, vp, vp, vp, f32, i32, i32, vp, i32, i32, i64, vp]),
    "lt_softargmax3d_bwd_dense": (C.c_int, [vp, vp, vp, vp, vp, vp, vp, vp, f32, i32, i32, vp, i32, i32, i64, vp]),
    "lt_volumetric_ce_fwd": (C.c_int, [vp, vp, vp, vp, vp, vp, vp, i32, i32, i64, vp]),
    "lt_bn_stats_workspace": (C.c_size_t, [i64, i32]),
    "lt_bn_stats_fwd": (C.c_int, [i32, vp, i64, i32, vp, vp, vp, vp, f32, vp, vp]),
    "lt_graph_begin": (C.c_int, [vp]),
    "lt_graph_end": (C.c_int, [vp, C.POINTER(vp)]),
    "lt_graph_launch": (C.c_int, [vp, vp]),
    "lt_graph_destroy": (C.c_int, [vp]),
    "lt_event_create": (C.c_int, [C.POINTER(vp)]),
    "lt_event_record": (C.c_int, [vp, vp]),
# ... 112 lines not shown
```

learnable-triangulation-pytorch_amd/mvn/models/pose_resnet.py:

```python
import torch
import torch.nn as nn

import lt_engine as E
import lt_hip as H

BN_MOMENTUM = 0.1

resnet_spec = {18: ("basic", [2, 2, 2, 2]), 34: ("basic", [3, 4, 6, 3]), 50: ("bottleneck", [3, 4, 6, 3]),
               101: ("bottleneck", [3, 4, 23, 3]), 152: ("bottleneck", [3, 8, 36, 3])}


def _bn(c):
    return nn.BatchNorm2d(c, momentum=BN_MOMENTUM)


def bn_tuple(bn):
    return E.BnParams(bn)


class ResidualBlock(nn.Module):

    def __init__(self, kind, inplanes, planes, stride=1, downsample=None, caffe=False):
        super().__init__()
        self.kind, self.stride = kind, stride
        if kind == "bottleneck":
            s1, s2 = (stride, 1) if caffe else (1, stride)
            shapes = [(inplanes, planes, 1, s1), (planes, planes, 3, s2), (planes, planes * 4, 1, 1)]
        else:
            shapes = [(inplanes, planes, 3, stride), (planes, planes, 3, 1)]
        self.strides = [s for _, _, _, s in shapes]
        for i, (ci, co, k, s) in enumerate(shapes, 1):
            setattr(self, "conv%d" % i, nn.Conv2d(ci, co, k, s, k // 2, bias=False))
            setattr(self, "bn%d" % i, _bn(co))
        self.downsample = downsample

    expansion = property(lambda self: 4 if self.kind == "bottleneck" else 1)

    def is_identity_bottleneck(self):
        return self.kind == "bottleneck" and self.downsample is None and all(s == 1 for s in self.strides)

    def record(self, b, x, t1=None, next_block=None):
        n = len(self.strides)
        if self.kind == "bottleneck" and self.downsample is None and t1 is None and next_block is None:
            convs = [self.conv1.weight, self.conv2.weight, self.conv3.weight]
            if b.can_bottleneck(x, convs, self.strides):
                return b.bottleneck(x, convs, [bn_tuple(self.bn1), bn_tuple(self.bn2), bn_tuple(self.bn3)])
        if self.kind == "bottleneck" and self.downsample is not None and t1 is None and next_block is None:
            convs = [self.conv1.weight, self.conv2.weight, self.conv3.weight]
            if b.can_bottleneck_ds(x, convs, self.strides, self.downsample[0].weight, self.downsample[0].stride[0]):
                return b.bottleneck_ds(x, convs, [bn_tuple(self.bn1), bn_tuple(self.bn2), bn_tuple(self.bn3)], self.downsample[0].weight,
                                       bn_tuple(self.downsample[1]))
        if t1 is not None or next_block is not None:
            assert self.is_identity_bottleneck()
            if t1 is None:
                t1 = b.conv(x, self.conv1.weight, None, bn_tuple(self.bn1), stride=1, pad=0, relu=True)
            t2 = b.conv(t1, self.conv2.weight, None, bn_tuple(self.bn2), stride=1, pad=1, relu=True)
            b.release(t1)
            if next_block is not None and b.can_expand_reduce(t2, x, self.conv3.weight, next_block.conv1.weight):
                y, t1n = b.expand_reduce(t2, x, self.conv3.weight, bn_tuple(self.bn3), next_block.conv1.weight, bn_tuple(next_block.bn1))
                b.release(t2)
                return y, t1n
            y = b.conv(t2, self.conv3.weight, None, bn_tuple(self.bn3), stride=1, pad=0, relu=True, residual=x)
            b.release(t2)
            return (y, None) if next_block is not None else y
        if self.kind == "bottleneck" and self.downsample is not None:
            ds, sds = self.downsample[0], self.downsample[0].stride[0]
            Ho, Wo = (x.shape[2] - 1) // sds + 1, (x.shape[3] - 1) // sds + 1
            if b.can_conv_cat2((x.shape[0], 1, Ho, Wo, self.conv3.weight.shape[1]), self.conv3.weight, x.shape, ds.weight, sds):
                t1 = b.conv(x, self.conv1.weight, None, bn_tuple(self.bn1), stride=self.conv1.stride[0], pad=0, relu=True)
                t2 = b.conv(t1, self.conv2.weight, None, bn_tuple(self.bn2), stride=self.conv2.stride[0], pad=1, relu=True)
                b.release(t1)
                y = b.conv_cat2(t2, self.conv3.weight, bn_tuple(self.bn3), x, ds.weight, bn_tuple(self.downsample[1]), sds)
                b.release(t2)
                return y
        res = x
        if self.downsample is not None:
            res = b.conv(x, self.downsample[0].weight, None, bn_tuple(self.downsample[1]), stride=self.downsample[0].stride[0], pad=0)
        y = x
        for i in range(1, n + 1):
            conv, bn = getattr(self, "conv%d" % i), getattr(self, "bn%d" % i)
            last = i == n
            z = b.conv(y, conv.weight, None, bn_tuple(bn), stride=conv.stride[0], pad=conv.padding[0], relu=True,
                       residual=res if last else None)
            if y is not x:
                b.release(y)
            y = z
        if res is not x:
            b.release(res)
        return y


class GlobalAveragePoolingHead(nn.Module):

    def __init__(self, in_channels, n_classes):
        super().__init__()
        self.features = nn.Sequential(
            nn.Conv2d(in_channels, 512, 3, stride=1, padding=1), _bn(512), nn.MaxPool2d(2), nn.ReLU(inplace=True),
            nn.Conv2d(512, 256, 3, stride=1, padding=1), _bn(256), nn.MaxPool2d(2), nn.ReLU(inplace=True))
        self.head = nn.Sequential(nn.Linear(256, 512), nn.ReLU(inplace=True), nn.Linear(512, 256), nn.ReLU(inplace=True),
                                  nn.Linear(256, n_classes), nn.Sigmoid())

    def record(self, b, x):
        f = self.features
        y = b.conv(x, f[0].weight, f[0].bias, bn_tuple(f[1]), stride=1, pad=1, relu=True)
        p = b.maxpool(y, 2, 2, 0, nd=2); b.release(y)
        y = b.conv(p, f[4].weight, f[4].bias, bn_tuple(f[5]), stride=1, pad=1, relu=True); b.release(p)
        p = b.maxpool(y, 2, 2, 0, nd=2); b.release(y)
        g = b.global_avgpool(p); b.release(p)
        h = self.head
        y = b.conv(g, h[0].weight[:, :, None, None], h[0].bias, None, relu=True); b.release(g)
        z = b.conv(y, h[2].weight[:, :, None, None], h[2].bias, None, relu=True); b.release(y)
        o = b.conv(z, h[4].weight[:, :, None, None], h[4].bias, None, sigmoid=True, out_f32=True); b.release(z)
        return o


class PoseResNet(E.PlanCache):
    def __init__(self, block_kind, layers, num_joints, num_input_channels=3, deconv_with_bias=False, num_deconv_layers=3,
                 num_deconv_filters=(256, 256, 256), num_deconv_kernels=(4, 4, 4), final_conv_kernel=1,
                 alg_confidences=False, vol_confidences=False, caffe=False):
        super().__init__()
        assert all(k == 4 for k in num_deconv_kernels), "only the 4x4 stride-2 deconvolution of the reference configs"
        self.num_joints, self.num_input_channels = num_joints, num_input_channels
        self.block_kind, self.caffe = block_kind, caffe
        exp = 4 if block_kind == "bottleneck" else 1
        self.conv1 = nn.Conv2d(num_input_channels, 64, kernel_size=7, stride=2, padding=3, bias=False)
        self.bn1 = _bn(64)
        inplanes = 64
        for li, (planes, nb) in enumerate(zip((64, 128, 256, 512), layers), 1):
            stride = 1 if li == 1 else 2
            blocks = []
            for bi in range(nb):
                st = stride if bi == 0 else 1
                ds = None
                if bi == 0 and (st != 1 or inplanes != planes * exp):
                    ds = nn.Sequential(nn.Conv2d(inplanes, planes * exp, kernel_size=1, stride=st, bias=False), _bn(planes * exp))
                blocks.append(ResidualBlock(block_kind, inplanes, planes, st, ds, caffe))
                inplanes = planes * exp
            setattr(self, "layer%d" % li, nn.Sequential(*blocks))
        if alg_confidences:
            self.alg_confidences = GlobalAveragePoolingHead(inplanes, num_joints)
        if vol_confidences:
            self.vol_confidences = GlobalAveragePoolingHead(inplanes, 32)
        dl = []
        for i in range(num_deconv_layers):
            dl += [nn.ConvTranspose2d(inplanes, num_deconv_filters[i], kernel_size=4, stride=2, padding=1, output_padding=0,
                                      bias=deconv_with_bias), _bn(num_deconv_filters[i]), nn.ReLU(inplace=True)]
            inplanes = num_deconv_filters[i]
        self.deconv_layers = nn.Sequential(*dl)
        self.final_layer = nn.Conv2d(inplanes, num_joints, kernel_size=final_conv_kernel, stride=1,
                                     padding=1 if final_conv_kernel == 3 else 0)
# ... 105 lines not shown
```

Baseline: 1485 samples/s.

## Fuse stride-2 downsampling bottleneck into one kernel with LDS-resident intermediates

Adds a single fused kernel for the layer2 first bottleneck (256->128->512, 3x3 stride 2, with a stride-2 projection shortcut). It computes conv1 over a halo tile, the strided 3x3 conv2 and a concatenated conv3+downsample GEMM entirely in LDS. This removes the separate conv1/conv2 launches and the global round-trips of t1/t2 that the conv_cat2 path still paid. In exchange it brings a large, register-heavy kernel with a DMA ring pipeline and a hard-coded shape gate. It also recomputes conv1 on halo pixels.

```diff
diff --git a/include/lt_hip.h b/include/lt_hip.h
--- a/include/lt_hip.h
+++ b/include/lt_hip.h
@@ -99,6 +99,7 @@
 int lt_sel_splitk_slices(const lt_conv_desc* d, const lt_wshape* w, int32_t transposed);
 int lt_sel_bottleneck(int32_t dtype, const int32_t x[5], const lt_wshape w[3], const int32_t strides[3]);
 int lt_sel_bottleneck_ds(int32_t dtype, const int32_t x[5], const lt_wshape w[3], const int32_t strides[3], const lt_wshape* w_down, int32_t stride_down);
+int lt_sel_bottleneck_s2(int32_t dtype, const int32_t x[5], const lt_wshape w[3], const int32_t strides[3], const lt_wshape* w_down, int32_t stride_down);
 int lt_sel_expand_reduce(int32_t dtype, const int32_t t2[5], const int32_t res[5], const lt_wshape* w_expand, const lt_wshape* w_reduce);
 int lt_sel_stem_pool(int32_t dtype, const int32_t x[5], const lt_wshape* w, int32_t stride, int32_t pad, const int32_t pool[3]);
 int lt_sel_pwchain(int32_t dtype, const int32_t x[5], int32_t nlayers, const lt_wshape* w);
@@ -305,6 +306,16 @@
 
 typedef struct {
     int32_t dtype;
+    int32_t N, H, W;
+    int32_t Cin, P, C;
+    const void* weight[3];
+    const float* scale[2];
+    const float* shift[3];
+} lt_bneck_s2_desc;
+int lt_bottleneck_s2_fwd(const lt_bneck_s2_desc* desc, const void* x, void* y, void* stream);
+
+typedef struct {
+    int32_t dtype;
     int32_t C, P;
     int64_t M;
     const void* weight[2];
@@ -353,6 +364,7 @@
     int32_t graph_captured;
     const float* logits;
     int32_t logits_planar;
+    int32_t n_bottleneck_s2;
 } lt_plan_info_t;
 int lt_plan_create_vol(const lt_vol_plan_config* cfg, const lt_named_tensor* weights, int32_t nweights, lt_plan** plan_out);
 int lt_plan_forward_vol(lt_plan* plan, const float* images, const double* K_host, const double* R_host, const double* t_host, const double* base_points_host,
diff --git a/learnable-triangulation-pytorch_amd/csrc/bneck.hip b/learnable-triangulation-pytorch_amd/csrc/bneck.hip
--- a/learnable-triangulation-pytorch_amd/csrc/bneck.hip
+++ b/learnable-triangulation-pytorch_amd/csrc/bneck.hip
@@ -729,6 +729,379 @@
     const long long nblk = (long long)a.N * a.tiles_x * a.tiles_y;
     hipLaunchKernelGGL(kern, dim3((unsigned)nblk), dim3(256), lds, s, a);
     LT_CHECK_LAUNCH("lt_bottleneck_ds_fwd");
+    return LT_OK;
+}
+
+
+struct BneckS2Args {
+    const bf16_t* x;
+    bf16_t* y;
+    const bf16_t* w1;
+    const bf16_t* w2;
+    const bf16_t* wcat;
+    const float* scale[2];
+    const float* shift[3];
+    int N, H, W, tiles_x, tiles_y;
+};
+
+#ifndef LT_S2_WD2
+#define LT_S2_WD2 6
+#endif
+#ifndef LT_S2_XD
+#define LT_S2_XD 1
+#endif
+#ifndef LT_S2_WD3
+#define LT_S2_WD3 6
+#endif
+
+#ifdef LT_BNECK_TRACE
+#define BN_STAMP8(k)                                                                                                        \
+    do {                                                                                                                    \
+        if (blockIdx.x < LT_BNECK_TRACE_WG / 2 && lane == 0) g_bneck_trace[(blockIdx.x * 8 + wave) * 8 + (k)] = clock64(); \
+    } while (0)
+#else
+#define BN_STAMP8(k)
+#endif
+
+template <int NK1, int AHEAD, int D, int NP>
+constexpr int bneck_after_np(int ks) {
+    int total = 0, last = 0;
+    for (int k = 0; k < D && k < NK1; ++k) { total += 2; if (k == ks) last = total; }
+    for (int k = 0; k < AHEAD && k < NK1; ++k) { total += NP; if (k == ks && total > last) last = total; }
+    for (int s = 0; s < ks; ++s) {
+        if (s + D < NK1) { total += 2; if (s + D == ks && total > last) last = total; }
+        if (s + AHEAD < NK1) { total += NP; if (s + AHEAD == ks && total > last) last = total; }
+    }
+    return total - last;
+}
+
+__global__ __launch_bounds__(512, 2) void bneck_s2_kernel(const BneckS2Args a) {
+    typedef bf16_t T;
+    constexpr int CIN = 256, P = 128, C = 512;
+    constexpr int TH = 8, TW = 8, HPI = 2 * TW + 1, HROWS = (2 * TH + 1) * HPI;
+    constexpr int NPB = 2;
+    constexpr int NCB = P / 32, NOB = C / 32, G2 = P / 16, GD = CIN / 16, NK1 = CIN / 32;
+    constexpr int RB = 2 * P;
+    constexpr int NPIECE = (HROWS + 15) / 16;
+    constexpr int STAGE = NPIECE * 1024, NST = 6, AHEAD = NST - 1;
+    constexpr int T1_BYTES = HROWS * RB, T2_OFF = 4 * STAGE, XS_OFF = NST * STAGE, XROW = 2 * CIN;
+    constexpr int NPB1 = 5, NOBW = NOB / 8;
+    static_assert(T1_BYTES <= T2_OFF && T2_OFF + NPB * 32 * RB <= XS_OFF, "t1 and t2 lie in the ring's bytes, the strided pixels of x behind it");
+    static_assert(T2_OFF % 256 == 0 && XS_OFF % 512 == 0 && STAGE % 256 == 0, "the XOR / bank arguments assume aligned regions");
+    static_assert(2 * NPB1 * 32 >= HROWS && NPIECE > 16 && NPIECE <= 24, "pixel blocks / pieces per wave");
+    constexpr int NP3 = NPIECE - 16;
+    auto fsw = [](int hr, int hc) -> int { return ((hc >> 1) & 7) | (((hr >> 1) & 1) << 3); };
+
+    extern __shared__ __attribute__((aligned(1024))) unsigned char smem[];
+    const unsigned lds0 = (unsigned)(size_t)(lptr_t)smem;
+    unsigned long long zp_bits = (unsigned long long)(size_t)g_zero_page_b;
+    asm volatile("" : "+s"(zp_bits));
+    const void* const zero_page = (const void*)(size_t)zp_bits;
+
+    const int t = threadIdx.x, lane = t & 63;
+    const int wave = __builtin_amdgcn_readfirstlane(t >> 6);
+    int lin = blockIdx.x;
+    {
+        const int nb = gridDim.x, q = nb >> 3, r = nb & 7, xcd = lin & 7, j = lin >> 3;
+        lin = (xcd < r ? xcd * (q + 1) : r * (q + 1) + (xcd - r) * q) + j;
+    }
+    const int tpi = a.tiles_x * a.tiles_y;
+    const int img = lin / tpi, rem = lin - img * tpi;
+    const int ty = rem / a.tiles_x, tx = rem - ty * a.tiles_x;
+    const int y0 = 2 * ty * TH - 1, x0 = 2 * tx * TW - 1;
+    const int Ho = a.H >> 1, Wo = a.W >> 1;
+    const T* __restrict__ x = a.x;
+
+    const int n31 = lane & 31, hk = lane >> 5;
+    const int cb = wave & 3, whalf = wave >> 2;
+    const int prr = n31 >> 3, pcc = n31 & 7;
+
+    float4 cst12;
+    float cst3;
+    {
+        const int l = lane & 31, arr = l >> 3, i4 = l & 7;
+        const float* t12 = arr == 0 ? a.scale[0] : arr == 1 ? a.shift[0] : arr == 2 ? a.scale[1] : a.shift[1];
+        cst12 = *(const float4*)(t12 + 32 * cb + 4 * i4);
+        cst3 = a.shift[2][32 * (wave + 8 * (lane >> 5)) + (lane & 31)];
+    }
+    auto cget = [&](const float4& tb, int f) -> float {
+        const float v = (f & 3) == 0 ? tb.x : (f & 3) == 1 ? tb.y : (f & 3) == 2 ? tb.z : tb.w;
+        return __int_as_float(__builtin_amdgcn_readlane(__float_as_int(v), f >> 2));
+    };
+    auto csel = [&](const float4& tb, int base, int e) -> float {
+        const float lo = cget(tb, base + 16 * (e >> 3) + (e & 7)), hi = cget(tb, base + 16 * (e >> 3) + 8 + (e & 7));
+        return hk ? hi : lo;
+    };
+    auto csel1 = [&](float v, int base, int e) -> float {
+        const float lo = __int_as_float(__builtin_amdgcn_readlane(__float_as_int(v), base + 16 * (e >> 3) + (e & 7)));
+        const float hi = __int_as_float(__builtin_amdgcn_readlane(__float_as_int(v), base + 16 * (e >> 3) + 8 + (e & 7)));
+        return hk ? hi : lo;
+    };
+
+    BN_STAMP8(0);
+    {
+#pragma unroll
+        for (int j = 0; j < 4; ++j) {
+            const int pc = wave + 8 * j, px = 2 * pc + (lane >> 5);
+            const int oy = px >> 3, ox = px & 7;
+            const int kvx = (lane & 31) ^ (px & 15);
+            dma16(x + (((size_t)(img * a.H + 2 * (ty * TH + oy)) * a.W + 2 * (tx * TW + ox)) * CIN + kvx * 8), lds0 + XS_OFF + pc * 1024);
+        }
+        const int prow = lane >> 2;
+        const int kvlog = (lane & 3) ^ swz64(prow);
+        int dbase[3];
+        bool dact[3];
+#pragma unroll
+        for (int i = 0; i < 3; ++i) {
+            const int hp = 16 * (wave + 8 * i) + prow;
+            const int hr = hp / HPI, hc = hp - hr * HPI;
+            const int iy = y0 + hr, ix = x0 + hc;
+            const bool ok = (hp < HROWS) & ((unsigned)iy < (unsigned)a.H) & ((unsigned)ix < (unsigned)a.W);
+            dbase[i] = ok ? ((img * a.H + iy) * a.W + ix) * CIN + kvlog * 8 : -1;
+            dact[i] = hp < HROWS;
+        }
+        const bool third = wave < NP3;
+        auto issue_piece = [&](int ks, unsigned stage_base, auto ic) {
+            constexpr int I = decltype(ic)::value;
+            if (I == 2 && !third) return;
+            if (dact[I]) {
+                const void* src = dbase[I] >= 0 ? (const void*)(x + (dbase[I] + ks * 32)) : zero_page;
+                dma16(src, lds0 + stage_base + (wave + 8 * I) * 1024);
+            }
+        };
+        const int hb0 = NPB1 * whalf;
+        const T* w1l = a.w1 + (size_t)cb * 512;
+        const unsigned wlane = lane * 16;
+        constexpr int DA = 3, NFA = DA + 1;
+        static_assert(AHEAD > DA && NK1 >= DA, "W1 prefetch distance");
+        V16 fa[NFA][2];
+        auto loadA = [&](int ks, V16 (&dst)[2]) {
+            const T* p = w1l + (size_t)(2 * ks) * NCB * 512;
+            gload16(dst[0], p, wlane);
+            gload16(dst[1], p + NCB * 512, wlane);
+        };
+        const unsigned fo0 = n31 * 64 + (((0 + hk) ^ swz64(n31)) << 4);
+        const unsigned fo1 = n31 * 64 + (((2 + hk) ^ swz64(n31)) << 4);
+
+        f32x16 acc[NPB1];
+#pragma unroll
+        for (int i = 0; i < NPB1; ++i)
+#pragma unroll
+            for (int e = 0; e < 16; ++e) acc[i][e] = 0.f;
+
+        static_for<0, DA>([&](auto kc) { loadA(decltype(kc)::value, fa[decltype(kc)::value]); });
+#pragma unroll
+        for (int s = 0; s < AHEAD; ++s)
+            static_for<0, 3>([&](auto ic) { issue_piece(s, s * STAGE, ic); });
+
+        static_for<0, NK1>([&](auto kc) {
+            constexpr int ks = decltype(kc)::value, R = ks % NFA;
+            constexpr unsigned rbuf = (ks % NST) * STAGE, wbuf = ((ks + AHEAD) % NST) * STAGE;
+            if (third) wait_vmcnt<bneck_after_np<NK1, AHEAD, DA, 3>(ks)>();
+            else wait_vmcnt<bneck_after_np<NK1, AHEAD, DA, 2>(ks)>();
+            asm volatile("s_waitcnt lgkmcnt(0)\n\ts_barrier" ::: "memory");
+            frag_ready(fa[R][0]);
+            frag_ready(fa[R][1]);
+            if constexpr (ks + DA < NK1) loadA(ks + DA, fa[(ks + DA) % NFA]);
+            if constexpr (ks + AHEAD < NK1) static_for<0, 3>([&](auto ic) { issue_piece(ks + AHEAD, wbuf, ic); });
+            const unsigned rb = lds0 + rbuf + hb0 * 2048;
+            V16 b0[NPB1], b1[NPB1];
+#pragma unroll
+            for (int i = 0; i < NPB1; ++i) b0[i].u = *(const uint4*)((lptr_t)(size_t)(rb + fo0 + i * 2048));
+            __builtin_amdgcn_sched_barrier(0);
+#pragma unroll
+            for (int i = 0; i < NPB1; ++i) b1[i].u = *(const uint4*)((lptr_t)(size_t)(rb + fo1 + i * 2048));
+#pragma unroll
+            for (int i = 0; i < NPB1; ++i) acc[i] = __builtin_amdgcn_mfma_f32_32x32x16_bf16(fa[R][0].h, b0[i].h, acc[i], 0, 0, 0);
+            __builtin_amdgcn_sched_barrier(0);
+#pragma unroll
+            for (int i = 0; i < NPB1; ++i) acc[i] = __builtin_amdgcn_mfma_f32_32x32x16_bf16(fa[R][1].h, b1[i].h, acc[i], 0, 0, 0);
+            __builtin_amdgcn_sched_barrier(0);
+        });
+        asm volatile("s_waitcnt vmcnt(0)\n\ts_waitcnt lgkmcnt(0)\n\ts_barrier" ::: "memory");
+        BN_STAMP8(1);
+
+        float esc[16], esf[16];
+#pragma unroll
+        for (int e = 0; e < 16; ++e) {
+            esc[e] = csel(cst12, 0, e);
+            esf[e] = csel(cst12, 32, e);
+        }
+#pragma unroll
+        for (int i = 0; i < NPB1; ++i) {
+            const int hp = 32 * (hb0 + i) + n31;
+            const int hr = hp / HPI, hc = hp - hr * HPI;
+            const int iy = y0 + hr, ix = x0 + hc;
+            const bool inimg = ((unsigned)iy < (unsigned)a.H) & ((unsigned)ix < (unsigned)a.W);
+            if (hp < HROWS) {
+#pragma unroll
+                for (int q = 0; q < 2; ++q) {
+                    unsigned o[4];
+#pragma unroll
+                    for (int d = 0; d < 4; ++d) {
+                        const int e = 8 * q + 2 * d;
+                        const float v0 = fmaxf(acc[i][e] * esc[e] + esf[e], 0.f), v1 = fmaxf(acc[i][e + 1] * esc[e + 1] + esf[e + 1], 0.f);
+                        o[d] = inimg ? pack_bf16x2(v0, v1) : 0u;
+                    }
+                    const int slot = (4 * cb + 2 * q + hk) ^ fsw(hr, hc);
+                    *(uint4*)((lptr_t)(size_t)(lds0 + hp * RB + slot * 16)) = make_uint4(o[0], o[1], o[2], o[3]);
+                }
+            }
+        }
+    }
+    __syncthreads();
+    BN_STAMP8(2);
+
+    constexpr int NUQ = G2 + GD, NU3 = NOBW * NUQ, WD3 = LT_S2_WD3;
+    const T* wl3 = a.wcat + (size_t)lane * 8;
+    auto load_w3 = [&](int u) -> V16 {
+        const int q = u / NUQ, k = u - q * NUQ;
+        V16 v;
+        v.u = *(const uint4*)(wl3 + ((size_t)k * NOB + wave + 8 * q) * 512);
+        return v;
+    };
+    V16 wf3[WD3 + 1];
+
+    if (wave < 4) {
+        constexpr int NPB2 = NPB;
+        const int bn = 2 * prr * HPI + 2 * pcc;
+        unsigned am[2][2];
+#pragma unroll
+        for (int cy = 0; cy < 2; ++cy)
+#pragma unroll
+            for (int cx = 0; cx < 2; ++cx) am[cy][cx] = lds0 + bn * RB + ((hk ^ (((pcc + cx) & 7) | (((prr + cy) & 1) << 3))) << 4);
+        const T* wl = a.w2 + ((size_t)cb * 64 + lane) * 8;
+        auto load_w = [&](int u) -> V16 {
+            V16 v;
+            v.u = *(const uint4*)(wl + (size_t)u * NCB * 512);
+            return v;
+        };
+        constexpr int NU = 9 * G2, WD = LT_S2_WD2, XD = LT_S2_XD;
+        V16 wf[WD + 1];
+#pragma unroll
+        for (int u = 0; u < WD; ++u) wf[u] = load_w(u);
+        f32x16 acc[NPB2];
+#pragma unroll
+        for (int i = 0; i < NPB2; ++i)
+#pragma unroll
+            for (int e = 0; e < 16; ++e) acc[i][e] = 0.f;
+        V16 xa[XD + 1][NPB2];
+        auto load_x = [&](auto uc, V16 (&dst)[NPB2]) {
+            constexpr int u = decltype(uc)::value;
+            constexpr int tap = u / G2, g = u % G2, dy = tap / 3, dx = tap % 3;
+            static_for<0, NPB2>([&](auto ic) {
+                constexpr int i = decltype(ic)::value;
+                constexpr int TT = (8 * i + dy) * HPI + dx;
+                const unsigned ad = am[dy >> 1][dx >> 1] ^ (g << 5);
+                dst[i].u = *(const uint4*)((lptr_t)(size_t)(ad + TT * RB));
+            });
+        };
+        static_for<0, XD>([&](auto uc) { load_x(uc, xa[decltype(uc)::value]); });
+        static_for<0, NU>([&](auto uc) {
+            constexpr int u = decltype(uc)::value;
+            if constexpr (u + WD < NU) wf[(u + WD) % (WD + 1)] = load_w(u + WD);
+            if constexpr (u + XD < NU) load_x(std::integral_constant<int, u + XD>{}, xa[(u + XD) % (XD + 1)]);
+#pragma unroll
+            for (int i = 0; i < NPB2; ++i)
+                acc[i] = __builtin_amdgcn_mfma_f32_32x32x16_bf16(wf[u % (WD + 1)].h, xa[u % (XD + 1)][i].h, acc[i], 0, 0, 0);
+            __builtin_amdgcn_sched_barrier(0);
+        });
+        BN_STAMP8(3);
+
+        float esc[16], esf[16];
+#pragma unroll
+        for (int e = 0; e < 16; ++e) {
+            esc[e] = csel(cst12, 64, e);
+            esf[e] = csel(cst12, 96, e);
+        }
+#pragma unroll
+        for (int i = 0; i < NPB2; ++i) {
+            const int px = 32 * i + n31;
+#pragma unroll
+            for (int q = 0; q < 2; ++q) {
+                unsigned o[4];
+#pragma unroll
+                for (int d = 0; d < 4; ++d) {
+                    const int e = 8 * q + 2 * d;
+                    o[d] = pack_bf16x2(fmaxf(acc[i][e] * esc[e] + esf[e], 0.f), fmaxf(acc[i][e + 1] * esc[e + 1] + esf[e + 1], 0.f));
+                }
+                const int slot = (4 * cb + 2 * q + hk) ^ (n31 & 15);
+                *(uint4*)((lptr_t)(size_t)(lds0 + T2_OFF + px * RB + slot * 16)) = make_uint4(o[0], o[1], o[2], o[3]);
+            }
+        }
+    }
+#pragma unroll
+    for (int u = 0; u < WD3; ++u) wf3[u] = load_w3(u);
+    __builtin_amdgcn_sched_barrier(0);
+    __syncthreads();
+    BN_STAMP8(4);
+
+    {
+        const unsigned a2 = lds0 + T2_OFF + n31 * RB + ((hk ^ (n31 & 15)) << 4);
+        const unsigned ax = lds0 + XS_OFF + n31 * XROW + ((hk ^ (n31 & 15)) << 4);
+        int poff[NPB];
+#pragma unroll
+        for (int pb = 0; pb < NPB; ++pb)
+            poff[pb] = ((img * Ho + ty * TH + 4 * pb + prr) * Wo + tx * TW + pcc) * C + 8 * hk;
+        f32x16 acc[NPB];
+        V16 xb[2][NPB];
+        auto load_b = [&](auto kc, V16 (&dst)[NPB]) {
+            constexpr int k = decltype(kc)::value;
+#pragma unroll
+            for (int pb = 0; pb < NPB; ++pb) {
+                if constexpr (k < G2) dst[pb].u = *(const uint4*)((lptr_t)(size_t)((a2 ^ (k << 5)) + pb * 32 * RB));
+                else dst[pb].u = *(const uint4*)((lptr_t)(size_t)((ax ^ ((k - G2) << 5)) + pb * 32 * XROW));
+            }
+        };
+        static_for<0, NU3>([&](auto uc) {
+            constexpr int u = decltype(uc)::value;
+            constexpr int q = u / NUQ, k = u % NUQ;
+            const int ob = wave + 8 * q;
+            if constexpr (k == 0) {
+#pragma unroll
+                for (int pb = 0; pb < NPB; ++pb)
+#pragma unroll
+                    for (int e = 0; e < 16; ++e) acc[pb][e] = 0.f;
+            }
+            if constexpr (u + WD3 < NU3) wf3[(u + WD3) % (WD3 + 1)] = load_w3(u + WD3);
+            if constexpr (u == 0) load_b(std::integral_constant<int, 0>{}, xb[0]);
+            if constexpr (u + 1 < NU3) load_b(std::integral_constant<int, (u + 1) % NUQ>{}, xb[(u + 1) & 1]);
+#pragma unroll
+            for (int pb = 0; pb < NPB; ++pb)
+                acc[pb] = __builtin_amdgcn_mfma_f32_32x32x16_bf16(wf3[u % (WD3 + 1)].h, xb[u & 1][pb].h, acc[pb], 0, 0, 0);
+            __builtin_amdgcn_sched_barrier(0);
+            if constexpr (k == NUQ - 1) {
+#pragma unroll
+                for (int j = 0; j < 2; ++j) {
+                    float esf[8];
+#pragma unroll
+                    for (int e = 0; e < 8; ++e) esf[e] = csel1(cst3, 32 * q, 8 * j + e);
+#pragma unroll
+                    for (int pb = 0; pb < NPB; ++pb) {
+                        unsigned o[4];
+#pragma unroll
+                        for (int d = 0; d < 4; ++d) {
+                            const int e = 2 * d;
+                            o[d] = pack_bf16x2(fmaxf(acc[pb][8 * j + e] + esf[e], 0.f), fmaxf(acc[pb][8 * j + e + 1] + esf[e + 1], 0.f));
+                        }
+                        *(uint4*)(a.y + poff[pb] + 32 * ob + 16 * j) = make_uint4(o[0], o[1], o[2], o[3]);
+                    }
+                }
+            }
+        });
+    }
+    BN_STAMP8(5);
+}
+
+constexpr int BNECK_S2_LDS = 6 * 19 * 1024 + 64 * 512;
+
+int launch_bneck_s2(const BneckS2Args& a, hipStream_t s) {
+    static_assert(BNECK_S2_LDS <= 160 * 1024, "one workgroup per CU");
+    auto kern = bneck_s2_kernel;
+    LT_OPT_IN_LDS(kern, BNECK_S2_LDS);
+    const long long nblk = (long long)a.N * a.tiles_x * a.tiles_y;
+    hipLaunchKernelGGL(kern, dim3((unsigned)nblk), dim3(512), BNECK_S2_LDS, s, a);
+    LT_CHECK_LAUNCH("lt_bottleneck_s2_fwd");
     return LT_OK;
 }
 
@@ -799,3 +1172,27 @@
     a.tiles_x = d->W / 16; a.tiles_y = d->H / 8;
     return launch_bneck_ds(a, (hipStream_t)stream);
 }
+
+extern "C" int lt_bottleneck_s2_fwd(const lt_bneck_s2_desc* d, const void* x, void* y, void* stream) {
+    LT_REQUIRE(d && x && y, LT_ERR_INVALID, "lt_bottleneck_s2_fwd: null argument");
+    LT_REQUIRE(x != y, LT_ERR_INVALID, "lt_bottleneck_s2_fwd: in-place is not possible");
+    LT_REQUIRE(d->dtype == LT_BF16, LT_ERR_UNSUPPORTED, "lt_bottleneck_s2_fwd: bf16 only");
+    LT_REQUIRE(d->Cin == 256 && d->P == 128 && d->C == 512, LT_ERR_UNSUPPORTED,
+               "lt_bottleneck_s2_fwd: widths %d -> %d -> %d (256 -> 128 -> 512: the first block of ResNet layer2)", d->Cin, d->P, d->C);
+    LT_REQUIRE(d->N > 0 && d->H > 0 && d->W > 0 && d->H % 16 == 0 && d->W % 16 == 0, LT_ERR_UNSUPPORTED,
+               "lt_bottleneck_s2_fwd: map %d x %d (16 x 16 pixel input tiles)", d->H, d->W);
+    LT_REQUIRE((long long)d->N * d->H * d->W * d->Cin < (1ll << 31), LT_ERR_UNSUPPORTED, "lt_bottleneck_s2_fwd: 32-bit element offsets");
+    BneckS2Args a;
+    a.x = (const bf16_t*)x;
+    a.y = (bf16_t*)y;
+    for (int i = 0; i < 3; ++i)
+        LT_REQUIRE(d->weight[i] && d->shift[i] && (i == 2 || d->scale[i]), LT_ERR_INVALID, "lt_bottleneck_s2_fwd: layer %d: null weight / scale / shift", i);
+    a.w1 = (const bf16_t*)d->weight[0];
+    a.w2 = (const bf16_t*)d->weight[1];
+    a.wcat = (const bf16_t*)d->weight[2];
+    a.scale[0] = d->scale[0]; a.scale[1] = d->scale[1];
+    a.shift[0] = d->shift[0]; a.shift[1] = d->shift[1]; a.shift[2] = d->shift[2];
+    a.N = d->N; a.H = d->H; a.W = d->W;
+    a.tiles_x = d->W / 16; a.tiles_y = d->H / 16;
+    return launch_bneck_s2(a, (hipStream_t)stream);
+}
diff --git a/learnable-triangulation-pytorch_amd/csrc/plan.hip b/learnable-triangulation-pytorch_amd/csrc/plan.hip
--- a/learnable-triangulation-pytorch_amd/csrc/plan.hip
+++ b/learnable-triangulation-pytorch_amd/csrc/plan.hip
@@ -248,6 +248,7 @@
     std::deque<lt_stem_desc> stem_descs;
     std::deque<lt_bneck_desc> bneck_descs;
     std::deque<lt_bneck_ds_desc> bneck_ds_descs;
+    std::deque<lt_bneck_s2_desc> bneck_s2_descs;
     std::deque<lt_xr_desc> xr_descs;
     hipGraphExec_t graph = nullptr;
     bool captured = false;
@@ -269,7 +270,7 @@
     std::vector<uint8_t> mask_cur;
     const uint8_t* mask_dev = nullptr; size_t o_mask = 0;
     uint8_t* amask_dev = nullptr; StagingRing amask;
-    int n_xr = 0, n_bneck = 0, n_bneck_ds = 0, n_cat2 = 0, n_halo2d = 0, n_pwchain = 0, n_stem = 0, n_splitk = 0, n_conv_skip = 0;
+    int n_xr = 0, n_bneck = 0, n_bneck_ds = 0, n_bneck_s2 = 0, n_cat2 = 0, n_halo2d = 0, n_pwchain = 0, n_stem = 0, n_splitk = 0, n_conv_skip = 0;
 
     ~lt_plan() {
         if (graph) (void)hipGraphExecDestroy(graph);
@@ -604,6 +605,39 @@
         ++n_bneck_ds;
         return LT_OK;
     }
+    int bottleneck_s2(const Act& x, const WT w[3], const BN bn[3], const WT& wd, const BN& bnd, Act& y) {
+        const int N = x.n, Hh = x.h, W = x.w, Cin = x.c, P = (int)w[0].s[0], Cc = (int)w[2].s[0], Ho = Hh / 2, Wo = W / 2;
+        PL_TRY(alloc(N, 1, Ho, Wo, Cc, es, y));
+        bneck_s2_descs.emplace_back();
+        lt_bneck_s2_desc& d = bneck_s2_descs.back();
+        memset(&d, 0, sizeof(d));
+        d.dtype = dtype; d.N = N; d.H = Hh; d.W = W; d.Cin = Cin; d.P = P; d.C = Cc;
+        const int xs[5] = {N, 1, Hh, W, Cin}, t1s[5] = {N, 1, Hh, W, P}, t2s[5] = {N, 1, Ho, Wo, P};
+        ConvSpec s1, s2, s3, sd_;
+        PL_TRY(pack_block_layer(w[0], bn[0], xs, 0, LT_EPI_RELU_POST, &d.weight[0], &d.scale[0], &d.shift[0], s1));
+        PL_TRY(pack_block_layer(w[1], bn[1], t1s, 1, LT_EPI_RELU_POST, &d.weight[1], &d.scale[1], &d.shift[1], s2));
+        flops -= 2.0 * N * ((double)Hh * W - (double)Ho * Wo) * P * 9 * P;
+        PL_TRY(make_conv_spec(w[2], nullptr, &bn[2], t2s, 1, 0, es, false, LT_EPI_RELU_POST, 0, s3));
+        PL_TRY(make_conv_spec(wd, nullptr, &bnd, xs, 2, 0, es, false, 0, 0, sd_));
+        LT_REQUIRE(s3.cout_pad == Cc && sd_.cout_pad == Cc, LT_ERR_INVALID, "plan: bottleneck_s2 widths");
+        const int kp = P + Cin;
+        std::vector<float> wcat((size_t)Cc * kp), shift(Cc);
+        for (int co = 0; co < Cc; ++co) {
+            for (int k = 0; k < P; ++k) wcat[(size_t)co * kp + k] = s3.ph[0].w[(size_t)co * s3.k_pad + k] * s3.scale[co];
+            for (int k = 0; k < Cin; ++k) wcat[(size_t)co * kp + P + k] = sd_.ph[0].w[(size_t)co * sd_.k_pad + k] * sd_.scale[co];
+            const float a = s3.bias[co] * s3.scale[co], a2 = a + s3.shift[co], b = sd_.bias[co] * sd_.scale[co], b2 = b + sd_.shift[co];
+            shift[co] = a2 + b2;
+        }
+        const void* wdev; PL_TRY(upload_w(wcat, &wdev));
+        PL_TRY(pack_frag(wdev, (size_t)Cc * kp, 2, Cc, kp, kp, 1, &d.weight[2]));
+        PL_TRY(upload_f32(shift, &d.shift[2]));
+        flops += 2.0 * N * Ho * Wo * Cc * kp;
+        const lt_bneck_s2_desc* dp = &d; const void* xp = x.p; void* yp = y.p;
+        ops.push_back([=](hipStream_t s) { return lt_bottleneck_s2_fwd(dp, xp, yp, s); });
+        ++n_bneck_s2;
+        ++n_cat2;
+        return LT_OK;
+    }
     int expand_reduce(const Act& t2, const Act& res, const WT& we, const BN& bne, const WT& wr, const BN& bnr, Act& y, Act& t1) {
         const int N = t2.n, Hh = t2.h, W = t2.w, P = t2.c, Cc = res.c;
         PL_TRY(alloc(N, 1, Hh, W, Cc, es, y));
@@ -687,6 +721,8 @@
             release(t2);
             return LT_OK;
         }
+        if (b.bottleneck && b.has_ds && lt_sel_bottleneck_s2(dtype, dims(x).data(), w3, b.strides, &wd, b.sds))
+            return bottleneck_s2(x, b.w, b.bn, b.wd, b.bnd, y);
         if (b.bottleneck && b.has_ds) {
             const int Ho = (x.h - 1) / b.sds + 1, Wo = (x.w - 1) / b.sds + 1;
             const int t2s[5] = {x.n, 1, Ho, Wo, (int)b.w[2].s[1]};
@@ -1396,7 +1432,7 @@
         info->flops += a.flops; info->bytes_allocated += a.bytes_allocated + (int64_t)p->bytes_alloc;
         info->n_expand_reduce += a.n_expand_reduce; info->n_bottleneck += a.n_bottleneck; info->n_bottleneck_ds += a.n_bottleneck_ds; info->n_conv_cat2 += a.n_conv_cat2;
         info->n_conv2d_halo += a.n_conv2d_halo; info->n_pwchain += a.n_pwchain; info->n_stem_pool += a.n_stem_pool; info->n_splitk += a.n_splitk;
-        info->n_conv_skip += a.n_conv_skip;
+        info->n_conv_skip += a.n_conv_skip; info->n_bottleneck_s2 += a.n_bottleneck_s2;
         info->graph_captured = (!p->sub_alg->cfg.use_graph || a.graph_captured) && (!p->sub_vol->cfg.use_graph || info->graph_captured) &&
                                (p->sub_alg->cfg.use_graph || p->sub_vol->cfg.use_graph) ? 1 : 0;
         return LT_OK;
@@ -1406,6 +1442,7 @@
     info->flops = p->flops; info->bytes_allocated = (int64_t)p->bytes_alloc;
     info->n_expand_reduce = p->n_xr; info->n_bottleneck = p->n_bneck; info->n_bottleneck_ds = p->n_bneck_ds; info->n_conv_cat2 = p->n_cat2;
     info->n_conv2d_halo = p->n_halo2d; info->n_pwchain = p->n_pwchain; info->n_stem_pool = p->n_stem; info->n_splitk = p->n_splitk; info->n_conv_skip = p->n_conv_skip;
+    info->n_bottleneck_s2 = p->n_bneck_s2;
     info->graph_captured = p->captured ? 1 : 0;
     info->logits = (const float*)p->logits.p; info->logits_planar = p->logits.planar ? 1 : 0;
     return LT_OK;
diff --git a/learnable-triangulation-pytorch_amd/csrc/select.hip b/learnable-triangulation-pytorch_amd/csrc/select.hip
--- a/learnable-triangulation-pytorch_amd/csrc/select.hip
+++ b/learnable-triangulation-pytorch_amd/csrc/select.hip
@@ -79,6 +79,19 @@
     return x[2] % 8 == 0 && x[3] % 16 == 0 && (long long)x[0] * x[2] * x[3] * 256 < (1ll << 31);
 }
 
+extern "C" int lt_sel_bottleneck_s2(int32_t dtype, const int32_t x[5], const lt_wshape w[3], const int32_t strides[3], const lt_wshape* wd, int32_t sd) {
+    if (dtype != LT_BF16 || env_on("LT_NO_BNECK") || env_on("LT_NO_BNECK_S2")) return 0;
+    if (x[1] != 1 || strides[0] != 1 || strides[1] != 2 || strides[2] != 1 || sd != 2) return 0;
+    if (x[4] != 256 || !wshape_is(&w[0], 4, 128, 256, 1, 1) || !wshape_is(&w[1], 4, 128, 128, 3, 3) || !wshape_is(&w[2], 4, 512, 128, 1, 1) ||
+        !wshape_is(wd, 4, 512, 256, 1, 1))
+        return 0;
+    if (x[2] % 16 || x[3] % 16 || (long long)x[0] * x[2] * x[3] * 256 >= (1ll << 31)) return 0;
+    const int32_t t2[5] = {x[0], 1, x[2] / 2, x[3] / 2, 128};
+    if (!lt_sel_conv_cat2(dtype, t2, &w[2], x, wd, sd)) return 0;
+    const long long tiles = (long long)x[0] * (x[2] / 16) * (x[3] / 16);
+    return tiles >= 256 || env_on("LT_BNECK_S2_ANY_SIZE");
+}
+
 extern "C" int lt_sel_expand_reduce(int32_t dtype, const int32_t t2[5], const int32_t res[5], const lt_wshape* we, const lt_wshape* wr) {
     if (dtype != LT_BF16 || env_on("LT_NO_XR")) return 0;
     if (t2[1] != 1 || res[1] != 1 || t2[0] != res[0] || t2[2] != res[2] || t2[3] != res[3] || res[4] != 1024 || t2[4] != 256) return 0;
diff --git a/learnable-triangulation-pytorch_amd/lt_engine.py b/learnable-triangulation-pytorch_amd/lt_engine.py
--- a/learnable-triangulation-pytorch_amd/lt_engine.py
+++ b/learnable-triangulation-pytorch_amd/lt_engine.py
@@ -204,7 +204,7 @@
     def _declines(self, *a, **k):
         return False
 
-    can_conv_skip = can_conv_cat2 = can_chain_pointwise = can_bottleneck = can_bottleneck_ds = can_expand_reduce = can_stem_pool = _declines
+    can_conv_skip = can_conv_cat2 = can_chain_pointwise = can_bottleneck = can_bottleneck_ds = can_bottleneck_s2 = can_expand_reduce = can_stem_pool = _declines
 
 
 class PlanBuilder(Recorder):
@@ -564,6 +564,45 @@
         assert self.can_bottleneck_ds(x, convs, (1, 1, 1), w_down, 1)
         return self._bneck(x, convs, bns, (w_down, bn_down))
 
+    def can_bottleneck_s2(self, x, convs, strides, w_down, stride_down):
+        if not self._fusable() or len(convs) != 3:
+            return False
+        return bool(H.lib().lt_sel_bottleneck_s2(self.code, H.dims(x.shape), (H.WShape * 3)(*map(H.wshape, convs)), H.i3(strides), H.wshape(w_down),
+                                                  stride_down))
+
+    def bottleneck_s2(self, x, convs, bns, w_down, bn_down):
+        assert self.can_bottleneck_s2(x, convs, (1, 2, 1), w_down, 2)
+        N, _, Hh, W, Cin = x.shape
+        P, Cc = convs[0].shape[0], convs[2].shape[0]
+        Ho, Wo = Hh // 2, W // 2
+        y = self.alloc((N, 1, Ho, Wo, Cc))
+        d = H.BneckS2Desc()
+        d.dtype, d.N, d.H, d.W, d.Cin, d.P, d.C = self.code, N, Hh, W, Cin, P, Cc
+        flops0 = self.flops
+        s1, d.weight[0], d.scale[0], d.shift[0] = self._pack_layer(convs[0], bns[0], x.shape, 0, H.EPI_RELU_POST)
+        s2p, d.weight[1], d.scale[1], d.shift[1] = self._pack_layer(convs[1], bns[1], (N, 1, Hh, W, P), 1, H.EPI_RELU_POST)
+        self.flops -= 2 * N * (Hh * W - Ho * Wo) * P * 9 * P
+        s2 = make_conv_spec(convs[1], None, bns[1], (N, 1, Hh, W, P), 2, 1, self.dtype, False, H.EPI_RELU_POST)
+        s3 = make_conv_spec(convs[2], None, bns[2], (N, 1, Ho, Wo, P), 1, 0, self.dtype, False, H.EPI_RELU_POST)
+        sd = make_conv_spec(w_down, None, bn_down, x.shape, 2, 0, self.dtype, False, 0)
+        assert s3.cout_pad == sd.cout_pad == Cc and s2p.Cout == s2.Cout == P
+        wcat = torch.cat([s3.phases[0].weight[:, :P] * s3.scale[:, None], sd.phases[0].weight[:, :Cin] * sd.scale[:, None]], dim=1).to(self.dtype)
+        shift = (s3.bias * s3.scale + s3.shift) + (sd.bias * sd.scale + sd.shift)
+        kp = P + Cin
+        scat = ConvSpec(N, 1, Ho, Wo, kp, 1, Ho, Wo, (1, 1, 1), (0, 0, 0), 1, Ho, Wo, (1, 1, 1), Cc, Cc, kp, H.EPI_RELU_POST, torch.zeros(Cc), torch.ones(Cc), shift)
+        wfr, _ = self._frag_copy(self.const(wcat, self.dtype), 2, scat, 1)
+        shd = self.const(shift)
+        d.weight[2], d.shift[2] = wfr.data_ptr(), shd.data_ptr()
+        self.flops += 2 * N * Ho * Wo * Cc * kp
+        self.keep += [x.t, d]
+        flops = self.flops - flops0
+        esz = x.t.element_size()
+        nbytes = (x.t.numel() + y.t.numel() + P * Cin + 9 * P * P + Cc * kp) * esz
+        label = "bneck-s2 %d->%d->%d @%s (expand + stride-2 downsample)" % (Cin, P, Cc, "x".join(str(v) for v in (N, 1, Hh, W)))
+        self._add(lambda s, d=d, xp=x.t.data_ptr(), yp=y.t.data_ptr(): H.check(self.lib.lt_bottleneck_s2_fwd(C.byref(d), xp, yp, s), "lt_bottleneck_s2_fwd"),
+                  "conv", label, flops, nbytes, {"bneck_ds": True, "bneck_s2": True, "specs": [s1, s2, s3, sd], "x": x, "y": y})
+        return y
+
     def can_expand_reduce(self, t2, res, w_expand, w_reduce):
         if not self._fusable():
             return False
diff --git a/learnable-triangulation-pytorch_amd/lt_hip.py b/learnable-triangulation-pytorch_amd/lt_hip.py
--- a/learnable-triangulation-pytorch_amd/lt_hip.py
+++ b/learnable-triangulation-pytorch_amd/lt_hip.py
@@ -83,6 +83,11 @@
                 ("weight", vp * 4), ("scale", vp * 4), ("shift", vp * 4)]
 
 
+class BneckS2Desc(C.Structure):
+    _fields_ = [("dtype", i32), ("N", i32), ("H", i32), ("W", i32), ("Cin", i32), ("P", i32), ("C", i32),
+                ("weight", vp * 3), ("scale", vp * 2), ("shift", vp * 3)]
+
+
 class XrDesc(C.Structure):
     _fields_ = [("dtype", i32), ("C", i32), ("P", i32), ("M", C.c_int64), ("weight", vp * 2), ("scale", vp * 2), ("shift", vp * 2), ("consts", vp)]
 
@@ -110,7 +115,8 @@
 class PlanInfo(C.Structure):
     _fields_ = [("launches", i32), ("heatmap_h", i32), ("heatmap_w", i32), ("flops", C.c_double), ("bytes_allocated", C.c_int64),
                 ("n_expand_reduce", i32), ("n_bottleneck", i32), ("n_bottleneck_ds", i32), ("n_conv_cat2", i32), ("n_conv2d_halo", i32), ("n_pwchain", i32),
-                ("n_stem_pool", i32), ("n_splitk", i32), ("n_conv_skip", i32), ("graph_captured", i32), ("logits", vp), ("logits_planar", i32)]
+                ("n_stem_pool", i32), ("n_splitk", i32), ("n_conv_skip", i32), ("graph_captured", i32), ("logits", vp), ("logits_planar", i32),
+                ("n_bottleneck_s2", i32)]
 
 
 SIGNATURES = {
@@ -139,6 +145,7 @@
     "lt_sel_splitk_slices": (C.c_int, [C.POINTER(ConvDesc), C.POINTER(WShape), i32]),
     "lt_sel_bottleneck": (C.c_int, [i32, i32 * 5, WShape * 3, i32 * 3]),
     "lt_sel_bottleneck_ds": (C.c_int, [i32, i32 * 5, WShape * 3, i32 * 3, C.POINTER(WShape), i32]),
+    "lt_sel_bottleneck_s2": (C.c_int, [i32, i32 * 5, WShape * 3, i32 * 3, C.POINTER(WShape), i32]),
     "lt_sel_expand_reduce": (C.c_int, [i32, i32 * 5, i32 * 5, C.POINTER(WShape), C.POINTER(WShape)]),
     "lt_sel_stem_pool": (C.c_int, [i32, i32 * 5, C.POINTER(WShape), i32, i32, i32 * 3]),
     "lt_sel_pwchain": (C.c_int, [i32, i32 * 5, i32, C.POINTER(WShape)]),
@@ -150,6 +157,7 @@
     "lt_stem_pool_fwd": (C.c_int, [C.POINTER(StemDesc), vp, vp, vp]),
     "lt_bottleneck_fwd": (C.c_int, [C.POINTER(BneckDesc), vp, vp, vp]),
     "lt_bottleneck_ds_fwd": (C.c_int, [C.POINTER(BneckDsDesc), vp, vp, vp]),
+    "lt_bottleneck_s2_fwd": (C.c_int, [C.POINTER(BneckS2Desc), vp, vp, vp]),
     "lt_expand_reduce_fwd": (C.c_int, [C.POINTER(XrDesc), vp, vp, vp, vp, vp]),
     "lt_stem_packed_bytes": (C.c_size_t, []),
     "lt_stem_pack_weights": (C.c_int, [vp, i32, vp, vp]),
diff --git a/learnable-triangulation-pytorch_amd/mvn/models/pose_resnet.py b/learnable-triangulation-pytorch_amd/mvn/models/pose_resnet.py
--- a/learnable-triangulation-pytorch_amd/mvn/models/pose_resnet.py
+++ b/learnable-triangulation-pytorch_amd/mvn/models/pose_resnet.py
@@ -65,7 +65,10 @@
             return (y, None) if next_block is not None else y
         if self.kind == "bottleneck" and self.downsample is not None:
             ds, sds = self.downsample[0], self.downsample[0].stride[0]
-            Ho, Wo = (x.shape[2] - 1) // sds + 1, (x.shape[3] - 1) // sds + 1
+            convs = [self.conv1.weight, self.conv2.weight, self.conv3.weight]
+            if b.can_bottleneck_s2(x, convs, self.strides, ds.weight, sds):
+                return b.bottleneck_s2(x, convs, [bn_tuple(self.bn1), bn_tuple(self.bn2), bn_tuple(self.bn3)], ds.weight, bn_tuple(self.downsample[1]))
+            Ho, Wo =(x.shape[2] - 1) // sds + 1, (x.shape[3] - 1) // sds + 1
             if b.can_conv_cat2((x.shape[0], 1, Ho, Wo, self.conv3.weight.shape[1]), self.conv3.weight, x.shape, ds.weight, sds):
                 t1 = b.conv(x, self.conv1.weight, None, bn_tuple(self.bn1), stride=self.conv1.stride[0], pad=0, relu=True)
                 t2 = b.conv(t1, self.conv2.weight, None, bn_tuple(self.bn2), stride=self.conv2.stride[0], pad=1, relu=True)
```

Result: no change. 1489 samples/s, median of 5 (+0.3%).
